# mhauskn/dqn-hfo

Hardware: AMD Instinct MI355X
Metric: DQN updates/sec, 1v0 HFO, 4x1024 MLP, minibatch 256 (higher is better)
Workload: dtype f32; 1 GPU; BASELINE configs[1]: 1v0 HFO, 1 MI355X, 4x1024 actor-critic, minibatch 256, 1M-transition device replay; replay_transitions=1000000, state_size=58, minibatch=256, minibatch_per_gpu=256, global_minibatch=256, parallelism=single, hip_graph=True, prewarm_updates=992, tuning_flags=0, sampling=on-device Philox, uniform with replacement

## Files before the change

### dqn-hfo_amd/capi.py

```python
import ctypes as C
import os

from ._build import LIB, build

MAX_HIDDEN = 8
DP_ID_BYTES = 128
DP_PER_LAYER, DP_HALF_GRADS, DP_SHARD_OPT = 1, 2, 4
DP_UNVERIFIED_OK = 256
TUNE_FP16_WGRAD_PER_LAYER = 1
TUNE_SEPARATE_HEAD_SEED = 2
TUNE_BWD_UNSHIFTED = 4
TUNE_SEPARATE_ACTOR_HEAD_BWD = 8
TUNE_SEPARATE_Q_TRAIN = 16
TUNE_SEPARATE_FIRST_LAYER = 32
TUNE_SEPARATE_CRITIC_FIRST_LAYERS = 64
TUNE_LATE_GATHER = 128
PLAN_FORMS = ("fp16", "data_parallel", "bwd_shifted_critic", "bwd_shifted_actor", "head_wgrad_rides_critic", "head_wgrad_rides_actor",
              "q_train_in_dgrad", "head_seed_fused", "dqda_head_bwd", "critic_l0_rides", "first_layers_merged", "early_gather_l0", "dp_tails_ride", "prioritized")
LOSS_SCALE_STATIC, LOSS_SCALE_DYNAMIC = 0, 1
FP32, FP16 = 0, 1
ACTOR, CRITIC, ACTOR_TARGET, CRITIC_TARGET = 0, 1, 2, 3
KIND_W, KIND_M, KIND_V, KIND_G = 0, 1, 2, 3
SOLVERS = ("Adam", "SGD", "Nesterov", "AdaGrad", "RMSProp", "AdaDelta")


class Config(C.Structure):
    _fields_ = [
        ("struct_size", C.c_int32), ("minibatch", C.c_int32), ("state_size", C.c_int32),
        ("num_hidden", C.c_int32), ("hidden", C.c_int32 * MAX_HIDDEN),
        ("replay_capacity", C.c_int32), ("soft_update_freq", C.c_int32),
        ("gamma", C.c_double), ("beta", C.c_double), ("tau", C.c_double),
        ("actor_lr", C.c_float), ("critic_lr", C.c_float), ("momentum", C.c_float),
        ("momentum2", C.c_float), ("delta", C.c_float), ("clip_gradients", C.c_float),
        ("device", C.c_int32), ("dp_world", C.c_int32), ("dp_rank", C.c_int32), ("use_graph", C.c_int32),
        ("seed", C.c_uint64), ("stream", C.c_void_p), ("grad_arena", C.c_void_p),
        ("grad_arena_bytes", C.c_size_t), ("precision", C.c_int32), ("loss_scale", C.c_float),
        ("solver_type", C.c_int32), ("rms_decay", C.c_float),
        ("tuning_flags", C.c_int32),
        ("loss_scale_mode", C.c_int32), ("loss_scale_growth_interval", C.c_int32),
        ("loss_scale_min_mult", C.c_float), ("loss_scale_max_mult", C.c_float),
    ]


class LossScaleState(C.Structure):
    _fields_ = [("struct_size", C.c_int32), ("mode", C.c_int32), ("mult_critic", C.c_float), ("mult_actor", C.c_float),
                ("good_critic", C.c_int32), ("good_actor", C.c_int32), ("backoffs_critic", C.c_int32), ("backoffs_actor", C.c_int32),
                ("growths_critic", C.c_int32), ("growths_actor", C.c_int32), ("skipped_steps", C.c_int32), ("reserved", C.c_int32)]


class UpdatePlan(C.Structure):
    _fields_ = [("struct_size", C.c_int32), ("forms", C.c_int32), ("launches_single", C.c_int32), ("launches_graph_first", C.c_int32),
                ("launches_in_graph", C.c_int32), ("updates_per_graph", C.c_int32), ("collectives", C.c_int32), ("solver_type", C.c_int32)]


class PerConfig(C.Structure):
    _fields_ = [("struct_size", C.c_int32), ("alpha", C.c_float), ("beta0", C.c_float), ("beta_anneal_iters", C.c_int32),
                ("eps", C.c_float), ("seed", C.c_uint64)]


class PerState(C.Structure):
    _fields_ = [("struct_size", C.c_int32), ("enabled", C.c_int32), ("levels", C.c_int32), ("size", C.c_int32),
                ("total", C.c_float), ("p_max", C.c_float), ("beta_now", C.c_float), ("reserved", C.c_float),
                ("next_counter", C.c_uint64), ("syncs", C.c_int64)]


class StateInfo(C.Structure):
    _fields_ = [("struct_size", C.c_int32), ("version", C.c_int32), ("flags", C.c_int32), ("precision", C.c_int32), ("minibatch", C.c_int32),
                ("state_size", C.c_int32), ("num_hidden", C.c_int32), ("hidden", C.c_int32 * MAX_HIDDEN), ("replay_capacity", C.c_int32),
                ("memory_size", C.c_int32), ("actor_iter", C.c_int32), ("critic_iter", C.c_int32), ("has_memory", C.c_int32),
                ("has_per", C.c_int32), ("has_loss_scale", C.c_int32), ("seed", C.c_uint64), ("update_counter", C.c_uint64),
                ("user_bytes", C.c_uint64), ("file_bytes", C.c_uint64), ("solver_type", C.c_int32), ("rms_decay", C.c_float)]


STATE_NO_MEMORY = 1

DIAG_BINS = 64
DIAG_MAX_BLOBS = 2 * (2 * MAX_HIDDEN + 4)
DIAG_MAX_PANELS = 5 * MAX_HIDDEN


class DiagMoments(C.Structure):
    _fields_ = [("count", C.c_int64), ("n_zero", C.c_int64), ("n_nonfinite", C.c_int64), ("sum_abs", C.c_double), ("sum_sq", C.c_double),
                ("max_abs", C.c_float), ("reserved", C.c_float)]


class DiagBlob(C.Structure):
    _fields_ = [("net", C.c_int32), ("layer", C.c_int32), ("is_bias", C.c_int32), ("reserved", C.c_int32),
                ("w", DiagMoments), ("g", DiagMoments), ("lag", DiagMoments), ("step", DiagMoments), ("g_hist", C.c_int32 * DIAG_BINS)]


class DiagPanel(C.Structure):
    _fields_ = [("pass_", C.c_int32), ("layer", C.c_int32), ("rows", C.c_int32), ("cols", C.c_int32), ("n_negative", C.c_int64),
                ("dead_units", C.c_int32), ("reserved", C.c_int32), ("a", DiagMoments), ("hist", C.c_int32 * DIAG_BINS)]


class DiagRow(C.Structure):
    _fields_ = [("min", C.c_float), ("max", C.c_float), ("sum", C.c_double), ("sum_sq", C.c_double), ("n_nonfinite", C.c_int64)]


class DiagAction(C.Structure):
    _fields_ = [("min", C.c_float), ("max", C.c_float), ("sum", C.c_double), ("n_out_of_bounds", C.c_int64)]


class DiagReport(C.Structure):
    _fields_ = [("struct_size", C.c_int32), ("n_blobs", C.c_int32), ("n_panels", C.c_int32), ("has_per", C.c_int32),
                ("blobs", DiagBlob * DIAG_MAX_BLOBS), ("panels", DiagPanel * DIAG_MAX_PANELS),
                ("q_target", DiagRow), ("y", DiagRow), ("q_train", DiagRow), ("q_policy", DiagRow), ("td", DiagRow),
                ("n_terminal", C.c_int64), ("actor_out", DiagAction * 10),
                ("dq_da_sum_abs", C.c_double), ("dq_da_max_abs", C.c_float), ("per_w_min", C.c_float), ("per_w_sum", C.c_double),
                ("per_prob_min", C.c_float), ("per_td_abs_max", C.c_float), ("actor_iter", C.c_int32), ("critic_iter", C.c_int32),
                ("critic_loss", C.c_float), ("avg_q", C.c_float), ("grad_norm", C.c_double * 2), ("clip_scale", C.c_double * 2),
                ("fp16", C.c_int32), ("loss_scale_mode", C.c_int32), ("loss_scale_critic", C.c_float), ("loss_scale_dqda", C.c_float),
                ("loss_scale_actor", C.c_float), ("mult_critic", C.c_float), ("mult_actor", C.c_float), ("reserved", C.c_int32)]

fp = C.POINTER(C.c_float)
ip = C.POINTER(C.c_int32)
up = C.POINTER(C.c_uint8)
H = C.c_void_p

SIGNATURES = {
    "dqnhip_default_config": (None, [C.POINTER(Config), C.c_int32]),
    "dqnhip_solver_name": (C.c_char_p, [C.c_int32]),
    "dqnhip_grad_arena_bytes": (C.c_size_t, [C.POINTER(Config)]),
    "dqnhip_last_error": (C.c_char_p, []),
    "dqnhip_create": (C.c_int, [C.POINTER(Config), C.POINTER(H)]),
    "dqnhip_destroy": (C.c_int, [H]),
    "dqnhip_update": (C.c_int, [H, ip, fp, fp]),
    "dqnhip_update_chained": (C.c_int, [H, ip, ip, fp, fp]),
    "dqnhip_update_async": (C.c_int, [H, ip]),
    "dqnhip_update_async_n": (C.c_int, [H, C.c_int32]),
    "dqnhip_update_pipelined": (C.c_int, [H, ip, fp, fp]),
    "dqnhip_update_indexed_n": (C.c_int, [H, ip, C.c_int32]),
    "dqnhip_collect_stats": (C.c_int, [H, fp, fp, C.c_int32, ip]),
    "dqnhip_benchmark_blocking": (C.c_int, [H, C.c_int32, C.c_int32, C.c_uint64, C.c_int32, fp]),
    "dqnhip_update_phase": (C.c_int, [H, C.c_int32, ip]),
    "dqnhip_update_abort": (C.c_int, [H]),
    "dqnhip_apply_update": (C.c_int, [H, C.c_int32]),
    "dqnhip_apply_update_sharded": (C.c_int, [H, C.c_int32, C.c_int32]),
    "dqnhip_get_update_plan": (C.c_int, [H, C.POINTER(UpdatePlan)]),
    "dqnhip_grad_buffer": (C.c_int, [H, C.c_int32, C.POINTER(C.c_void_p), C.POINTER(C.c_size_t)]),
    "dqnhip_read_stats": (C.c_int, [H, fp, fp]),
    "dqnhip_dp_unique_id": (C.c_int, [C.c_void_p, C.c_size_t]),
    "dqnhip_dp_init": (C.c_int, [H, C.c_void_p, C.c_size_t, C.c_int32]),
    "dqnhip_dp_init_file": (C.c_int, [H, C.c_char_p, C.c_int32, C.c_int32]),
    "dqnhip_dp_rendezvous_file": (C.c_int, [C.c_char_p, C.c_int32, C.c_int32, C.c_int32, C.c_void_p, C.c_size_t]),
    "dqnhip_dp_rendezvous_cleanup": (C.c_int, [C.c_char_p, C.c_int32]),
    "dqnhip_dp_graph_active": (C.c_int, [H, ip]),
    "dqnhip_dp_broadcast_params": (C.c_int, [H, C.c_int32]),
    "dqnhip_dp_update": (C.c_int, [H, ip]),
    "dqnhip_dp_update_n": (C.c_int, [H, C.c_int32]),
    "dqnhip_dp_gather_state": (C.c_int, [H]),
    "dqnhip_dp_destroy": (C.c_int, [H]),
    "dqnhip_dp_info": (C.c_int, [ip, C.c_char_p, C.c_size_t]),
    "dqnhip_skipped_steps": (C.c_int, [H, C.POINTER(C.c_int64)]),
    "dqnhip_get_loss_scale": (C.c_int, [H, C.POINTER(LossScaleState)]),
    "dqnhip_set_loss_scale": (C.c_int, [H, C.c_float, C.c_float]),
    "dqnhip_reduce_gradients_local": (C.c_int, [C.POINTER(H), C.c_int32, C.c_int32]),
    "dqnhip_sample_states": (C.c_int, [H, ip, C.c_int32, fp]),
    "dqnhip_get_actor_output": (C.c_int, [H, C.c_int32, C.c_int32, fp]),
    "dqnhip_files_matching_regexp": (C.c_int, [C.c_char_p, C.c_char_p, C.c_size_t, ip]),
    "dqnhip_remove_snapshots": (C.c_int, [C.c_char_p, C.c_int32]),
    "dqnhip_benchmark": (C.c_int, [H, C.c_int32, C.c_int32, fp]),
    "dqnhip_select_actions": (C.c_int, [H, fp, C.c_int32, fp]),
    "dqnhip_select_actions_device": (C.c_int, [H, C.c_void_p, C.c_int32, C.c_void_p]),
    "dqnhip_select_actions_net": (C.c_int, [H, C.c_int32, fp, C.c_int32, fp]),
    "dqnhip_critic_forward": (C.c_int, [H, C.c_int32, fp, fp, C.c_int32, fp]),
    "dqnhip_set_act_precision": (C.c_int, [H, C.c_int32]),
    "dqnhip_get_act_precision": (C.c_int, [H, ip]),
    "dqnhip_add_transitions": (C.c_int, [H, fp, fp, fp, fp, fp, up, C.c_int32]),
    "dqnhip_add_transition": (C.c_int, [H, fp, fp, C.c_float, C.c_float, fp, C.c_uint8]),
    "dqnhip_add_transitions_device": (C.c_int, [H, C.c_void_p, C.c_void_p, C.c_void_p, C.c_void_p,
                                                C.c_void_p, C.c_void_p, C.c_int32]),
    "dqnhip_label_transitions": (C.c_int, [C.c_double, fp, C.c_int32, fp]),
    "dqnhip_memory_size": (C.c_int, [H, ip]),
    "dqnhip_clear_memory": (C.c_int, [H]),
    "dqnhip_read_memory": (C.c_int, [H, C.c_int32, C.c_int32, fp, fp, fp, fp, fp, up]),
    "dqnhip_snapshot_replay_memory": (C.c_int, [H, C.c_char_p]),
    "dqnhip_load_replay_memory": (C.c_int, [H, C.c_char_p]),
    "dqnhip_get_config": (C.c_int, [H, C.POINTER(Config)]),
    "dqnhip_save_caffemodel": (C.c_int, [H, C.c_int32, C.c_char_p]),
    "dqnhip_load_caffemodel": (C.c_int, [H, C.c_int32, C.c_char_p]),
    "dqnhip_solver_snapshot": (C.c_int, [H, C.c_int32, C.c_char_p, ip]),
    "dqnhip_solver_restore": (C.c_int, [H, C.c_int32, C.c_char_p]),
    "dqnhip_snapshot": (C.c_int, [H, C.c_char_p, C.c_char_p, C.c_int32, C.c_int32]),
    "dqnhip_snapshot_async": (C.c_int, [H, C.c_char_p, C.c_char_p, C.c_int32, C.c_int32, C.c_int32]),
    "dqnhip_snapshot_wait": (C.c_int, [H, C.POINTER(C.c_int32), C.POINTER(C.c_int32)]),
    "dqnhip_snapshot_poll": (C.c_int, [H, C.POINTER(C.c_int32)]),
    "dqnhip_find_latest_snapshot": (C.c_int, [C.c_char_p, C.c_char_p, C.c_char_p, C.c_char_p, C.c_size_t]),
    "dqnhip_find_hiscore": (C.c_int, [C.c_char_p, ip]),
    "dqnhip_remove_files_matching_regexp": (C.c_int, [C.c_char_p]),
    "dqnhip_param_count": (C.c_int, [H, C.c_int32, C.POINTER(C.c_size_t)]),
    "dqnhip_get_params": (C.c_int, [H, C.c_int32, C.c_int32, fp, C.c_size_t]),
    "dqnhip_set_params": (C.c_int, [H, C.c_int32, C.c_int32, fp, C.c_size_t]),
    "dqnhip_clone_to_target": (C.c_int, [H, C.c_int32]),
    "dqnhip_share_parameters": (C.c_int, [H, H, C.c_int32, C.c_int32]),
    "dqnhip_share_replay_memory": (C.c_int, [H, H]),
    "dqnhip_get_iters": (C.c_int, [H, ip, ip]),
    "dqnhip_set_iters": (C.c_int, [H, C.c_int32, C.c_int32]),
    "dqnhip_debug_read": (C.c_int, [H, C.c_char_p, fp, C.c_size_t]),
    "dqnhip_get_stream": (C.c_int, [H, C.POINTER(C.c_void_p)]),
    "dqnhip_set_kernel_timing": (C.c_int, [H, C.c_int32]),
    "dqnhip_get_kernel_timing": (C.c_int, [H, C.c_char_p, fp, C.POINTER(C.c_int64), C.c_int32]),
    "dqnhip_diag_collect": (C.c_int, [H, C.POINTER(DiagReport)]),
    "dqnhip_per_default_config": (None, [C.POINTER(PerConfig)]),
    "dqnhip_per_enable": (C.c_int, [H, C.POINTER(PerConfig)]),
    "dqnhip_per_get_state": (C.c_int, [H, C.POINTER(PerState)]),
    "dqnhip_per_get_priorities": (C.c_int, [H, C.c_int32, C.c_int32, fp]),
    "dqnhip_per_set_priorities": (C.c_int, [H, C.c_int32, C.c_int32, fp]),
    "dqnhip_per_sample": (C.c_int, [H, C.c_uint64, C.c_int32, ip, fp]),
    "dqnhip_per_debug_read": (C.c_int, [H, C.c_char_p, fp, C.c_size_t]),
    "dqnhip_save_state": (C.c_int, [H, C.c_char_p, C.c_int32, C.c_void_p, C.c_size_t]),
    "dqnhip_load_state": (C.c_int, [H, C.c_char_p]),
    "dqnhip_state_info": (C.c_int, [C.c_char_p, C.POINTER(StateInfo)]),
    "dqnhip_state_read_user": (C.c_int, [C.c_char_p, C.c_void_p, C.c_size_t, C.POINTER(C.c_size_t)]),
    "dqnhip_save_state_async": (C.c_int, [H, C.c_char_p, C.c_int32, C.c_void_p, C.c_size_t]),
    "dqnhip_save_state_wait": (C.c_int, [H]),
    "dqnhip_save_state_poll": (C.c_int, [H, C.POINTER(C.c_int32)]),
    "dqnhip_state_crc32_device": (C.c_int, [H, C.c_void_p, C.c_size_t, C.c_int32, C.POINTER(C.c_uint32)]),
}

class EnvConfig(C.Structure):
    _fields_ = [("struct_size", C.c_int32), ("workers", C.c_int32), ("max_steps", C.c_int32), ("unum", C.c_int32),
                ("p_end", C.c_float), ("p_goal", C.c_float), ("seed", C.c_uint64)]


SIGNATURES.update({
    "dqnhip_env_create": (C.c_int, [H, C.POINTER(EnvConfig), C.POINTER(C.c_void_p)]),
    "dqnhip_env_destroy": (C.c_int, [C.c_void_p]),
    "dqnhip_env_step": (C.c_int, [C.c_void_p, C.c_float, C.c_int32]),
    "dqnhip_env_stats": (C.c_int, [C.c_void_p, C.POINTER(C.c_int64), C.POINTER(C.c_int64), C.POINTER(C.c_double),
                                   C.POINTER(C.c_int64)]),
    "dqnhip_env_debug_read": (C.c_int, [C.c_void_p, C.c_char_p, fp, C.c_size_t]),
})

ENV_NO_RECORD = 1


class EnvEpisode(C.Structure):
    _fields_ = [("total_reward", C.c_double), ("extrinsic_reward", C.c_double), ("steps", C.c_int32), ("status", C.c_int32),
                ("worker", C.c_int32), ("reserved", C.c_int32), ("step_index", C.c_int64)]


SIGNATURES.update({
    "dqnhip_env_create_external": (C.c_int, [H, C.POINTER(EnvConfig), C.c_int32, fp, C.POINTER(C.c_void_p)]),
    "dqnhip_env_act": (C.c_int, [C.c_void_p, C.c_float, ip, fp, fp]),
    "dqnhip_env_act_device": (C.c_int, [C.c_void_p, C.c_float, C.c_void_p, C.c_void_p, C.c_void_p]),
    "dqnhip_env_observe": (C.c_int, [C.c_void_p, fp, ip, ip]),
    "dqnhip_env_observe_device": (C.c_int, [C.c_void_p, C.c_void_p, C.c_void_p, C.c_void_p]),
    "dqnhip_env_read_episodes": (C.c_int, [C.c_void_p, C.POINTER(EnvEpisode), C.c_int32, ip, C.POINTER(C.c_int64)]),
})

_lib = None


def load(rebuild=False):
    global _lib
    if _lib is None or rebuild:
        build()
        if not os.path.exists(LIB):
            raise RuntimeError("libdqnhip.so is missing: the HIP extension is mandatory")
        lib = C.CDLL(LIB)
        for name, (res, args) in SIGNATURES.items():
            fn = getattr(lib, name)
            fn.restype = res
            fn.argtypes = args
        _lib = lib
    return _lib
```

### dqn-hfo_amd/csrc/gemm_bodies.hip.h

```cpp
#pragma once
#include <hip/hip_runtime.h>

#include <cstdint>

#include "learner_args.hip.h"

namespace dqnhip {


__host__ __device__ __forceinline__ void tile_of_counts(int tiles_p, int tiles_q, int b, int& tile_p, int& tile_q) {
  const bool xmap = (tiles_p & 7) == 0;
  const int j = xmap ? b >> 3 : b;
  const int d = j / tiles_q;
  tile_q = j - d * tiles_q;
  tile_p = xmap ? d * 8 + (b & 7) : d;
}
constexpr int kTileDecodeMaxQ = 1024, kTileDecodeMaxTiles = 1 << 18;
__host__ __device__ __forceinline__ uint32_t tile_magic(int tiles_q) { return (uint32_t)((0x80000000ull + (uint32_t)tiles_q - 1) / (uint32_t)tiles_q); }
__host__ __device__ __forceinline__ bool tile_magic_covers(int tiles_p, int tiles_q) {
  return tiles_p >= 1 && tiles_q >= 1 && tiles_q <= kTileDecodeMaxQ && (int64_t)tiles_p * tiles_q <= kTileDecodeMaxTiles;
}
__host__ __device__ __forceinline__ void tile_decode(int tiles_p, int tiles_q, uint32_t magic, int b, int& tile_p, int& tile_q) {
  const bool xmap = (tiles_p & 7) == 0;
  const int j = xmap ? b >> 3 : b;
  const int d = (int)(((uint64_t)(2u * (uint32_t)j + 1u) * magic) >> 32);
  tile_q = j - d * tiles_q;
  tile_p = xmap ? d * 8 + (b & 7) : d;
}
__device__ __forceinline__ void tile_of_problem(const GemmProblem& pr, int b, int& tile_p, int& tile_q) {
  tile_of_counts(pr.tiles_p, pr.tiles_q, b, tile_p, tile_q);
}
__device__ __forceinline__ void tile_of_block(const GemmBatch& batch, int& pi, int& tile_p, int& tile_q) {
  int b = blockIdx.x;
  pi = 0;
#pragma unroll
  for (int i = 1; i < kMaxGroup; ++i)
    if (i < batch.n && b >= batch.prob[i].tile_base) pi = i;
  const GemmProblem& pr = batch.prob[pi];
  tile_of_problem(pr, b - pr.tile_base, tile_p, tile_q);
}

__device__ __forceinline__ GemmProblem make_problem(const float* P, const float* Q, float* C, int ldp, int ldq, int ldc, int Pdim, int Qdim, int Kred,
                                                    int mode, const GemmCold& c, int tiles_p, int tiles_q, int tile_base) {
  GemmProblem pr;
  pr.P = P; pr.ldp = ldp; pr.Q = Q; pr.ldq = ldq; pr.C = C; pr.ldc = ldc; pr.Pdim = Pdim; pr.Qdim = Qdim; pr.Kred = Kred;
  pr.bias = c.bias; pr.mask = c.mask; pr.ldm = c.ldm; pr.db = c.db; pr.partial = c.partial; pr.relu = c.relu;
  pr.seed_w = c.seed_w; pr.C2 = c.C2; pr.dot_w = c.dot_w; pr.dot_out = c.dot_out;
  pr.xcopy_dst = c.xcopy_dst; pr.xcopy_col = c.xcopy_col; pr.xcopy_n = c.xcopy_n;
  pr.mode = mode; pr.tiles_p = tiles_p; pr.tiles_q = tiles_q; pr.tile_base = tile_base;
  return pr;
}
template <int N>
struct HotArgs { GemmHeader hd; GemmHot hot[N]; };
template <int N>
__device__ __forceinline__ int request_args(const GemmArgs<N>& a, HotArgs<N>& r, int b, int x0 = 0, int x1 = 0) {
  r.hd = a.head;
#pragma unroll
  for (int i = 0; i < N; ++i) r.hot[i] = a.hot[i];
  const GemmHot &h0 = r.hot[0], &h1 = r.hot[N > 1 ? 1 : 0], &h2 = r.hot[N > 2 ? 2 : 0], &h3 = r.hot[N > 3 ? 3 : 0];
  asm volatile("" : "+s"(b) : "s"(r.hd.tile_base[1]), "s"(r.hd.tiles_p[0]), "s"(r.hd.tiles_q[0]), "s"(x0), "s"(x1),
               "s"(h0.P), "s"(h0.ldp), "s"(h0.C), "s"(h1.P), "s"(h1.ldp), "s"(h1.C), "s"(h2.P), "s"(h2.ldp), "s"(h2.C), "s"(h3.P), "s"(h3.ldp), "s"(h3.C),
               "s"(h0.Pdim), "s"(h1.Pdim), "s"(h2.Pdim), "s"(h3.Pdim), "s"(h0.tq_magic), "s"(h1.tq_magic), "s"(h2.tq_magic), "s"(h3.tq_magic));
  return b;
}
template <int I, int N>
__device__ __forceinline__ GemmProblem problem_at(const GemmArgs<N>& a, const HotArgs<N>& r) {
  static_assert(I < N, "record not carried");
  const GemmHot& h = r.hot[I];
  return make_problem(h.P, h.Q, h.C, h.ldp, h.ldq, h.ldc, h.Pdim, h.Qdim, h.Kred, h.mode, a.cold[I], r.hd.tiles_p[I], r.hd.tiles_q[I], r.hd.tile_base[I]);
}
template <int I, int N>
__device__ __forceinline__ void tile_of_record(const HotArgs<N>& r, int b, int& tile_p, int& tile_q) {
  static_assert(I < N, "record not carried");
  tile_decode(r.hd.tiles_p[I], r.hd.tiles_q[I], r.hot[I].tq_magic, b, tile_p, tile_q);
}
template <int N>
__device__ __forceinline__ GemmProblem problem_of_tile(const GemmArgs<N>& a, const HotArgs<N>& r, const int b, int& tile_p, int& tile_q) {
  const GemmHeader& hd = r.hd;
  int pi = 0;
  int tiles_p = hd.tiles_p[0], tiles_q = hd.tiles_q[0], tile_base = hd.tile_base[0];
  GemmHot h = r.hot[0];
  if (N > 1 && b >= hd.tile_base[N > 1 ? 1 : 0]) {
    pi = 1;
    tiles_p = hd.tiles_p[N > 1 ? 1 : 0]; tiles_q = hd.tiles_q[N > 1 ? 1 : 0]; tile_base = hd.tile_base[N > 1 ? 1 : 0];
    h = r.hot[N > 1 ? 1 : 0];
    if (N > 2 && b >= hd.tile_base[N > 2 ? 2 : 0]) {
      constexpr int I2 = N > 2 ? 2 : 0, I3 = N > 3 ? 3 : I2;
      const bool last = N > 3 && b >= hd.tile_base[I3];
      const GemmHot &h2 = r.hot[I2], &h3 = r.hot[I3];
      pi = last ? I3 : I2;
      tiles_p = last ? hd.tiles_p[I3] : hd.tiles_p[I2]; tiles_q = last ? hd.tiles_q[I3] : hd.tiles_q[I2];
      tile_base = last ? hd.tile_base[I3] : hd.tile_base[I2];
      h.P = last ? h3.P : h2.P; h.Q = last ? h3.Q : h2.Q; h.C = last ? h3.C : h2.C;
      h.ldp = last ? h3.ldp : h2.ldp; h.ldq = last ? h3.ldq : h2.ldq; h.ldc = last ? h3.ldc : h2.ldc;
      h.Pdim = last ? h3.Pdim : h2.Pdim; h.Qdim = last ? h3.Qdim : h2.Qdim; h.Kred = last ? h3.Kred : h2.Kred;
      h.mode = last ? h3.mode : h2.mode; h.tq_magic = last ? h3.tq_magic : h2.tq_magic;
      asm volatile("" : "+s"(pi));
    }
    asm volatile("" : "+s"(pi));
  }
  tile_decode(tiles_p, tiles_q, h.tq_magic, b - tile_base, tile_p, tile_q);
  return make_problem(h.P, h.Q, h.C, h.ldp, h.ldq, h.ldc, h.Pdim, h.Qdim, h.Kred, h.mode, a.cold[N == 1 ? 0 : pi], tiles_p, tiles_q, tile_base);
}
template <int N>
__device__ __forceinline__ GemmProblem problem_of_block(const GemmArgs<N>& a, int& tile_p, int& tile_q) {
  HotArgs<N> r;
  const int b = request_args(a, r, (int)blockIdx.x);
  return problem_of_tile(a, r, b, tile_p, tile_q);
}

template <int NACC>
__device__ __forceinline__ void park_accumulators(float* smem, const f32x4 (&acc)[NACC], int wave, int lane) {
  f32x4* s = reinterpret_cast<f32x4*>(smem);
#pragma unroll
  for (int e = 0; e < NACC; ++e) s[(wave * NACC + e) * 64 + lane] = acc[e];
}
template <int NACC>
__device__ __forceinline__ f32x4 reduce_accumulator(const float* smem, int e, int lane) {
  const f32x4* s = reinterpret_cast<const f32x4*>(smem);
  const f32x4 a0 = s[(0 * NACC + e) * 64 + lane], a1 = s[(1 * NACC + e) * 64 + lane];
  const f32x4 a2 = s[(2 * NACC + e) * 64 + lane], a3 = s[(3 * NACC + e) * 64 + lane];
  f32x4 r;
  r.x = (a0.x + a1.x) + (a2.x + a3.x); r.y = (a0.y + a1.y) + (a2.y + a3.y);
  r.z = (a0.z + a1.z) + (a2.z + a3.z); r.w = (a0.w + a1.w) + (a2.w + a3.w);
  return r;
}

#define DQN_MFMA(a, b, c) __builtin_amdgcn_mfma_f32_16x16x4f32((a), (b), (c), 0, 0, 0)
#define DQN_PIN() __builtin_amdgcn_sched_barrier(0)

__device__ __forceinline__ void store_head_seed(const GemmProblem& pr, int q, int p, const f32x4& v, const f32x4& sw) {
  f32x4 dz;
  dz.x = (-sw.x) * lrelu_mask(v.x); dz.y = (-sw.y) * lrelu_mask(v.y);
  dz.z = (-sw.z) * lrelu_mask(v.z); dz.w = (-sw.w) * lrelu_mask(v.w);
  *reinterpret_cast<f32x4*>(pr.C2 + (size_t)q * pr.ldc + p) = dz;
}

__device__ __forceinline__ void store_head_dot(const GemmProblem& pr, int q, int p, int lg, const f32x4& v, const f32x4& dw) {
  float d = fmaf(v.x, dw.x, 0.0f); d = fmaf(v.y, dw.y, d); d = fmaf(v.z, dw.z, d); d = fmaf(v.w, dw.w, d);
  d += __shfl_xor(d, 16, 64);
  d += __shfl_xor(d, 32, 64);
  if (lg == 0) pr.dot_out[(size_t)q * (pr.Pdim >> 4) + (p >> 4)] = d;
}

template <int TP, int TQ>
__device__ __forceinline__ void fwd_direct_body(const GemmProblem& pr, int tile_p, int tile_q, float* smem) {
  constexpr int NACC = TP * TQ;
  const int lane = threadIdx.x & 63, wave = threadIdx.x >> 6;
  const int li = lane & 15, lg = lane >> 4;
  const int p0 = tile_p * 16 * TP, q0 = tile_q * 16 * TQ;
  const int Kw = pr.Kred >> 2;
  const int nkb = Kw >> 4;
  const int wave_u = __builtin_amdgcn_readfirstlane(wave);
  const char* pp[TP];
  const char* qp[TQ];
  const uint32_t lofp = ((uint32_t)li * (uint32_t)pr.ldp + (uint32_t)lg * 4u) * 4u, lofq = ((uint32_t)li * (uint32_t)pr.ldq + (uint32_t)lg * 4u) * 4u;
#pragma unroll
  for (int c = 0; c < TP; ++c) pp[c] = c == 0 ? reinterpret_cast<const char*>(pr.P + (size_t)p0 * pr.ldp + wave_u * Kw) : pp[c > 0 ? c - 1 : 0] + (size_t)64 * pr.ldp;
#pragma unroll
  for (int a = 0; a < TQ; ++a) qp[a] = a == 0 ? reinterpret_cast<const char*>(pr.Q + (size_t)q0 * pr.ldq + wave_u * Kw) : qp[a > 0 ? a - 1 : 0] + (size_t)64 * pr.ldq;

  f32x4 acc[NACC];
#pragma unroll
  for (int e = 0; e < NACC; ++e) acc[e] = f32x4{0.f, 0.f, 0.f, 0.f};
  f32x4 rp[4][TP], rq[4][TQ];

#define FWD_LOAD(slot, kb)                                                              \
  {                                                                                     \
    _Pragma("unroll") for (int c = 0; c < TP; ++c)                                      \
        rp[slot][c] = *reinterpret_cast<const f32x4*>(pp[c] + ((kb) << 6) + lofp);     \
    _Pragma("unroll") for (int a = 0; a < TQ; ++a)                                      \
        rq[slot][a] = *reinterpret_cast<const f32x4*>(qp[a] + ((kb) << 6) + lofq);     \
  }
#define FWD_COMPUTE(slot)                                                               \
  {                                                                                     \
    _Pragma("unroll") for (int s = 0; s < 4; ++s)                                       \
    _Pragma("unroll") for (int a = 0; a < TQ; ++a)                                      \
    _Pragma("unroll") for (int c = 0; c < TP; ++c)                                      \
        acc[a * TP + c] = DQN_MFMA(rp[slot][c][s], rq[slot][a][s], acc[a * TP + c]);    \
  }

  const int nkb4 = nkb & ~3;
  if (nkb4 > 0) {
    FWD_LOAD(0, 0) FWD_LOAD(1, 1) FWD_LOAD(2, 2) FWD_LOAD(3, 3)
    int kb = 0;
    for (; kb + 4 < nkb4; kb += 4) {
      FWD_COMPUTE(0) DQN_PIN(); FWD_LOAD(0, kb + 4) DQN_PIN();
      FWD_COMPUTE(1) DQN_PIN(); FWD_LOAD(1, kb + 5) DQN_PIN();
      FWD_COMPUTE(2) DQN_PIN(); FWD_LOAD(2, kb + 6) DQN_PIN();
      FWD_COMPUTE(3) DQN_PIN(); FWD_LOAD(3, kb + 7) DQN_PIN();
    }
    FWD_COMPUTE(0) FWD_COMPUTE(1) FWD_COMPUTE(2) FWD_COMPUTE(3)
  }
  {
    const int rem = nkb - nkb4;
    if (rem > 0) FWD_LOAD(0, nkb4)
    if (rem > 1) FWD_LOAD(1, nkb4 + 1)
    if (rem > 2) FWD_LOAD(2, nkb4 + 2)
    if (rem > 0) FWD_COMPUTE(0)
    if (rem > 1) FWD_COMPUTE(1)
    if (rem > 2) FWD_COMPUTE(2)
  }
#undef FWD_LOAD
#undef FWD_COMPUTE

  constexpr int NBV = (NACC + 3) / 4;
  f32x4 bvp[NBV], swp[NBV], dwp[NBV];
  if (pr.bias != nullptr) {
#pragma unroll
    for (int j = 0; j < NBV; ++j) {
      const int e = j * 4 + wave;
      if (e < NACC) bvp[j] = *reinterpret_cast<const f32x4*>(pr.bias + p0 + (e % TP) * 16 + (lg << 2));
    }
  }
  if (pr.seed_w != nullptr) {
#pragma unroll
    for (int j = 0; j < NBV; ++j) {
      const int e = j * 4 + wave;
      if (e < NACC) swp[j] = *reinterpret_cast<const f32x4*>(pr.seed_w + p0 + (e % TP) * 16 + (lg << 2));
    }
  }
  if (pr.dot_w != nullptr) {
#pragma unroll
    for (int j = 0; j < NBV; ++j) {
      const int e = j * 4 + wave;
      if (e < NACC) dwp[j] = *reinterpret_cast<const f32x4*>(pr.dot_w + p0 + (e % TP) * 16 + (lg << 2));
    }
  }
  if (pr.xcopy_dst != nullptr && (int)threadIdx.x < 16 * TP) {
    const float* src = pr.P + (size_t)(p0 + threadIdx.x) * pr.ldp + pr.xcopy_col;
    for (int j = tile_q; j < pr.xcopy_n; j += pr.tiles_q) pr.xcopy_dst[(size_t)j * pr.Pdim + p0 + threadIdx.x] = src[j];
  }
  park_accumulators<NACC>(smem, acc, wave, lane);
  __syncthreads();
#pragma unroll
  for (int e = 0; e < NACC; ++e) {
    if ((e & 3) == wave) {
      const int a = e / TP, c = e % TP;
      f32x4 v = reduce_accumulator<NACC>(smem, e, lane);
      const int q = q0 + a * 16 + li, p = p0 + c * 16 + (lg << 2);
      if (pr.bias != nullptr) {
        const f32x4 bv = bvp[e >> 2];
        v.x += bv.x; v.y += bv.y; v.z += bv.z; v.w += bv.w;
      }
      if (pr.relu) { v.x = lrelu_fwd(v.x); v.y = lrelu_fwd(v.y); v.z = lrelu_fwd(v.z); v.w = lrelu_fwd(v.w); }
      *reinterpret_cast<f32x4*>(pr.C + (size_t)q * pr.ldc + p) = v;
      if (pr.seed_w != nullptr) store_head_seed(pr, q, p, v, swp[e >> 2]);
      if (pr.dot_w != nullptr) store_head_dot(pr, q, p, lg, v, dwp[e >> 2]);
    }
  }
}

template <int TPB, int TQ>
__device__ __forceinline__ void dgrad_direct_body(const GemmProblem& pr, int tile_p, int tile_q, float* smem) {
  constexpr int NACC = TPB * 4 * TQ;
  const int lane = threadIdx.x & 63, wave = threadIdx.x >> 6;
  const int li = lane & 15, lg = lane >> 4;
  const int p0 = tile_p * 64 * TPB, q0 = tile_q * 16 * TQ;
  const int Kw = pr.Kred >> 2;
  const int nkb = Kw >> 4;
  const float* pp = pr.P + (size_t)(wave * Kw + lg * 4) * pr.ldp + p0 + li * 4;
  const float* qp[TQ];
#pragma unroll
  for (int a = 0; a < TQ; ++a) qp[a] = pr.Q + (size_t)(q0 + a * 16 + li) * pr.ldq + wave * Kw + lg * 4;
  const size_t ldp = pr.ldp;

  f32x4 acc[NACC];
#pragma unroll
  for (int e = 0; e < NACC; ++e) acc[e] = f32x4{0.f, 0.f, 0.f, 0.f};
  f32x4 rp[4][4][TPB], rq[4][TQ];

#define DG_LOAD(slot, kb)                                                               \
  {                                                                                     \
    _Pragma("unroll") for (int a = 0; a < TQ; ++a)                                      \
        rq[slot][a] = *reinterpret_cast<const f32x4*>(qp[a] + ((kb) << 4));            \
    _Pragma("unroll") for (int s = 0; s < 4; ++s)                                       \
    _Pragma("unroll") for (int b = 0; b < TPB; ++b)                                     \
        rp[slot][s][b] = *reinterpret_cast<const f32x4*>(pp + (size_t)(((kb) << 4) + s) * ldp + b * 64); \
  }
#define DG_COMPUTE(slot)                                                                \
  {                                                                                     \
    _Pragma("unroll") for (int s = 0; s < 4; ++s)                                       \
    _Pragma("unroll") for (int a = 0; a < TQ; ++a)                                      \
    _Pragma("unroll") for (int b = 0; b < TPB; ++b)                                     \
    _Pragma("unroll") for (int pc = 0; pc < 4; ++pc)                                    \
        acc[(a * TPB + b) * 4 + pc] =                                                   \
            DQN_MFMA(rp[slot][s][b][pc], rq[slot][a][s], acc[(a * TPB + b) * 4 + pc]);  \
  }

  const int nkb4 = nkb & ~3;
  if (nkb4 > 0) {
    DG_LOAD(0, 0) DG_LOAD(1, 1) DG_LOAD(2, 2) DG_LOAD(3, 3)
    int kb = 0;
    for (; kb + 4 < nkb4; kb += 4) {
      DG_COMPUTE(0) DQN_PIN(); DG_LOAD(0, kb + 4) DQN_PIN();
      DG_COMPUTE(1) DQN_PIN(); DG_LOAD(1, kb + 5) DQN_PIN();
      DG_COMPUTE(2) DQN_PIN(); DG_LOAD(2, kb + 6) DQN_PIN();
      DG_COMPUTE(3) DQN_PIN(); DG_LOAD(3, kb + 7) DQN_PIN();
    }
    DG_COMPUTE(0) DG_COMPUTE(1) DG_COMPUTE(2) DG_COMPUTE(3)
  }
  for (int kb = nkb4; kb < nkb; ++kb) { DG_LOAD(0, kb) DG_COMPUTE(0) }
#undef DG_LOAD
#undef DG_COMPUTE

  constexpr int NMK = (TQ * TPB + 3) / 4;
  f32x4 mk[NMK][4];
  if (pr.mask != nullptr) {
#pragma unroll
    for (int j = 0; j < NMK; ++j) {
      const int ab = j * 4 + wave;
      if (ab < TQ * TPB) {
#pragma unroll
        for (int r = 0; r < 4; ++r)
          mk[j][r] = *reinterpret_cast<const f32x4*>(pr.mask + (size_t)(q0 + (ab / TPB) * 16 + li) * pr.ldm + p0 + (ab % TPB) * 64 + (lg << 4) + (r << 2));
      }
    }
  }
  park_accumulators<NACC>(smem, acc, wave, lane);
  __syncthreads();
#pragma unroll
  for (int ab = 0; ab < TQ * TPB; ++ab) {
    if ((ab & 3) == wave) {
      const int a = ab / TPB, b = ab % TPB;
      f32x4 r0 = reduce_accumulator<NACC>(smem, ab * 4 + 0, lane);
      f32x4 r1 = reduce_accumulator<NACC>(smem, ab * 4 + 1, lane);
      f32x4 r2 = reduce_accumulator<NACC>(smem, ab * 4 + 2, lane);
      f32x4 r3 = reduce_accumulator<NACC>(smem, ab * 4 + 3, lane);
      const int q = q0 + a * 16 + li;
#pragma unroll
      for (int r = 0; r < 4; ++r) {
        const int p = p0 + b * 64 + (lg << 4) + (r << 2);
        f32x4 v = f32x4{r0[r], r1[r], r2[r], r3[r]};
        if (pr.mask != nullptr) {
          const f32x4 mv = mk[ab >> 2][r];
          v.x *= lrelu_mask(mv.x); v.y *= lrelu_mask(mv.y); v.z *= lrelu_mask(mv.z); v.w *= lrelu_mask(mv.w);
        }
        *reinterpret_cast<f32x4*>(pr.C + (size_t)q * pr.ldc + p) = v;
      }
    }
  }
}

template <int NS = 4>
__device__ __forceinline__ f32x4 dgrad_narrow_tile(const GemmProblem& pr, int tile_p, int tile_q, float* smem) {
  constexpr int NACC = 1;
  const int lane = threadIdx.x & 63, wave = threadIdx.x >> 6;
  const int li = lane & 15, lg = lane >> 4;
  const int p0 = tile_p * 16, q0 = tile_q * 16;
  const int Kw = pr.Kred >> 2;
  const int nkb = Kw >> 4;
  const float* pp = pr.P + (size_t)(wave * Kw + lg * 4) * pr.ldp + p0 + li;
  const float* qp = pr.Q + (size_t)(q0 + li) * pr.ldq + wave * Kw + lg * 4;
  const size_t ldp = pr.ldp;
  f32x4 acc[NACC];
  acc[0] = f32x4{0.f, 0.f, 0.f, 0.f};
  float rp[NS][4]; f32x4 rq[NS];
#define DN_LOAD(slot, kb)                                                               \
  {                                                                                     \
    rq[slot] = *reinterpret_cast<const f32x4*>(qp + ((kb) << 4));                      \
    _Pragma("unroll") for (int s = 0; s < 4; ++s) rp[slot][s] = pp[(size_t)(((kb) << 4) + s) * ldp]; \
  }
#define DN_COMPUTE(slot)                                                                \
  { _Pragma("unroll") for (int s = 0; s < 4; ++s) acc[0] = DQN_MFMA(rp[slot][s], rq[slot][s], acc[0]); }
  const int nkbN = nkb - nkb % NS;
  if (nkbN > 0) {
#pragma unroll
    for (int i = 0; i < NS; ++i) { DN_LOAD(i, i) DQN_PIN(); }
    int kb = 0;
    for (; kb + NS < nkbN; kb += NS) {
#pragma unroll
      for (int i = 0; i < NS; ++i) { DN_COMPUTE(i) DQN_PIN(); DN_LOAD(i, kb + NS + i) DQN_PIN(); }
    }
#pragma unroll
    for (int i = 0; i < NS; ++i) { DN_COMPUTE(i) }
  }
  for (int kb = nkbN; kb < nkb; ++kb) { DN_LOAD(0, kb) DN_COMPUTE(0) }
#undef DN_LOAD
#undef DN_COMPUTE
  f32x4 mv = f32x4{0.f, 0.f, 0.f, 0.f};
  if (wave == 0 && pr.mask != nullptr) mv = *reinterpret_cast<const f32x4*>(pr.mask + (size_t)(q0 + li) * pr.ldm + p0 + (lg << 2));
  park_accumulators<NACC>(smem, acc, wave, lane);
  __syncthreads();
  f32x4 v = f32x4{0.f, 0.f, 0.f, 0.f};
  if (wave == 0) {
    v = reduce_accumulator<NACC>(smem, 0, lane);
    if (pr.mask != nullptr) {
      v.x *= lrelu_mask(mv.x); v.y *= lrelu_mask(mv.y); v.z *= lrelu_mask(mv.z); v.w *= lrelu_mask(mv.w);
    }
  }
  return v;
}
template <int NS = 4>
__device__ __forceinline__ f32x4 dgrad_narrow_tile16(const NarrowTile16& pr, int tile_q, float* smem) {
  typedef __attribute__((ext_vector_type(4))) _Float16 h4;
  const int lane = threadIdx.x & 63, wave = threadIdx.x >> 6;
  const int li = lane & 15, lg = lane >> 4;
  const int q0 = tile_q * 16;
  const int Kw = pr.Kred >> 2;
  const int nkb = Kw >> 4;
  const _Float16* pp = pr.P + (size_t)(wave * Kw + lg * 4) * pr.ldp + li;
  const _Float16* qp = pr.Q + (size_t)(q0 + li) * pr.ldq + wave * Kw + lg * 4;
  const size_t ldp = pr.ldp;
  f32x4 acc[1];
  acc[0] = f32x4{0.f, 0.f, 0.f, 0.f};
  _Float16 rp[NS][4]; h4 rq[NS];
#define DN_LOAD(slot, kb)                                                               \
  {                                                                                     \
    rq[slot] = *reinterpret_cast<const h4*>(qp + ((kb) << 4));                         \
    _Pragma("unroll") for (int s = 0; s < 4; ++s) rp[slot][s] = pp[(size_t)(((kb) << 4) + s) * ldp]; \
  }
// ... 617 lines not shown
```

### dqn-hfo_amd/csrc/gemm_common.hip.h

```cpp
#pragma once
#include <hip/hip_runtime.h>
#include <hip/hip_ext.h>
#include <stdint.h>

namespace dqnhip {

typedef float f32x4 __attribute__((ext_vector_type(4)));

enum GemmMode { GEMM_FWD = 0, GEMM_DGRAD = 1, GEMM_WGRAD = 2 };

constexpr float kLeakySlope = 0.01f;

struct GemmProblem {
  const float* P; int ldp;
  const float* Q; int ldq;
  float* C; int ldc;
  int Pdim, Qdim, Kred;
  const float* bias;
  const float* mask; int ldm;
  float* db;
  float* partial;
  int relu;
  const float* seed_w; float* C2;
  const float* dot_w; float* dot_out;
  float* xcopy_dst; int xcopy_col, xcopy_n;
  int mode;
  int tiles_p, tiles_q, tile_base;
};

constexpr int kMaxLeadingDim = 1 << 26;
constexpr int kMaxGroup = 4;
struct GemmBatch {
  GemmProblem prob[kMaxGroup];
  int n;
  int total_tiles;
};

struct alignas(64) GemmHeader {
  int tile_base[kMaxGroup];
  int tiles_p[kMaxGroup], tiles_q[kMaxGroup];
  int n, total_tiles, pad[2];
};
struct alignas(64) GemmHot {
  const float* P; const float* Q;
  int ldp, ldq, Kred, ldc;
  float* C;
  int mode;
  int Pdim, Qdim;
  uint32_t tq_magic;
  int pad[2];
};
struct GemmCold {
  const float* bias; const float* mask; float* db; float* partial;
  const float* seed_w; float* C2; const float* dot_w; float* dot_out; float* xcopy_dst;
  int ldm, relu, xcopy_col, xcopy_n;
};
template <int N>
struct GemmArgs {
  GemmHeader head;
  GemmHot hot[N];
  GemmCold cold[N];
};
static_assert(sizeof(GemmHeader) == 64 && sizeof(GemmHot) == 64, "one 16-dword scalar load each");

struct LaunchOn {
  hipStream_t stream;
  hipEvent_t start = nullptr, stop = nullptr;
  LaunchOn(hipStream_t s) : stream(s) {}
  LaunchOn(hipStream_t s, hipEvent_t t0, hipEvent_t t1) : stream(s), start(t0), stop(t1) {}
};
template <typename K, typename... A>
inline hipError_t launch(const LaunchOn& on, K kernel, dim3 grid, dim3 block, size_t lds, const A&... args) {
  if (on.start) hipExtLaunchKernelGGL(kernel, grid, block, (uint32_t)lds, on.stream, on.start, on.stop, 0, args...);
  else hipLaunchKernelGGL(kernel, grid, block, lds, on.stream, args...);
  return hipGetLastError();
}

__device__ __forceinline__ float lrelu_fwd(float x) {
  return fmaxf(x, 0.0f) + kLeakySlope * fminf(x, 0.0f);
}
__device__ __forceinline__ float lrelu_mask(float y) {
  return (y > 0.0f ? 1.0f : 0.0f) + kLeakySlope * (y <= 0.0f ? 1.0f : 0.0f);
}

__device__ __forceinline__ float wave_sum64(float v) {
  v += __builtin_bit_cast(float, __builtin_amdgcn_update_dpp(0, __builtin_bit_cast(int, v), 0xB1, 0xF, 0xF, false));
  v += __builtin_bit_cast(float, __builtin_amdgcn_update_dpp(0, __builtin_bit_cast(int, v), 0x4E, 0xF, 0xF, false));
  v += __builtin_bit_cast(float, __builtin_amdgcn_update_dpp(0, __builtin_bit_cast(int, v), 0x141, 0xF, 0xF, false));
  v += __builtin_bit_cast(float, __builtin_amdgcn_update_dpp(0, __builtin_bit_cast(int, v), 0x140, 0xF, 0xF, false));
  v += __builtin_bit_cast(float, __builtin_amdgcn_update_dpp(0, __builtin_bit_cast(int, v), 0x142, 0xA, 0xF, false));
  v += __builtin_bit_cast(float, __builtin_amdgcn_update_dpp(0, __builtin_bit_cast(int, v), 0x143, 0xC, 0xF, false));
  return __builtin_bit_cast(float, __builtin_amdgcn_readlane(__builtin_bit_cast(int, v), 63));
}

constexpr int kFlagTarget = 1;
constexpr int kFlagGradNorm = 2;

__device__ __forceinline__ float ls_live(float base, const float* mult) { return mult != nullptr ? base * *mult : base; }

struct TailsArgs {
  const float* loss_partial; int n_loss; const double* q_partial; int n_q;
  float inv_batch; float* critic_tail; float* actor_tail; const int* flags;
  int on;
};
__device__ __forceinline__ void tails_block(const TailsArgs& a, float* sdot , double* sq ) {
  const int t = threadIdx.x;
  float dot = 0.0f; double qs = 0.0;
  if (a.critic_tail != nullptr) for (int i = t; i < a.n_loss; i += 256) dot += a.loss_partial[i];
  if (a.actor_tail != nullptr) for (int i = t; i < a.n_q; i += 256) qs += a.q_partial[i];
#pragma unroll
  for (int off = 32; off > 0; off >>= 1) { dot += __shfl_xor(dot, off, 64); qs += __shfl_xor(qs, off, 64); }
  if ((t & 63) == 0) { sdot[t >> 6] = dot; sq[t >> 6] = qs; }
  __syncthreads();
  if (t != 0) return;
  if (a.critic_tail != nullptr) {
    dot = (sdot[0] + sdot[1]) + (sdot[2] + sdot[3]);
    a.critic_tail[0] = dot * a.inv_batch / 2.0f;
    a.critic_tail[1] = 0.f; a.critic_tail[2] = (*a.flags & kFlagTarget) ? 1.0f : 0.f; a.critic_tail[3] = 0.f;
  }
  if (a.actor_tail != nullptr) {
    qs = (sq[0] + sq[1]) + (sq[2] + sq[3]);
    a.actor_tail[0] = 0.f; a.actor_tail[1] = (float)qs; a.actor_tail[2] = 0.f; a.actor_tail[3] = 0.f;
  }
}

}
```

### dqn-hfo_amd/csrc/gemm_direct.hip.h

```cpp
#pragma once
#include <hip/hip_runtime.h>

#include <algorithm>
#include <cstdint>
#include <cstdlib>

#include "gemm_bodies.hip.h"
#include "gemm_plan.hip.h"

namespace dqnhip {

template <int TP, int TQ>
__global__ __launch_bounds__(256) void gemm_fwd_direct(const GemmArgs<kMaxGroup> args) {
  extern __shared__ __attribute__((aligned(16))) float smem[];
  int tile_p, tile_q;
  const GemmProblem pr = problem_of_block(args, tile_p, tile_q);
  fwd_direct_body<TP, TQ>(pr, tile_p, tile_q, smem);
}
template <int TP, int TQ, bool PIN, int NSLOT = 2>
__global__ __launch_bounds__(256) void gemm_fwd_lds(const GemmArgs<kMaxGroup> args) {
  extern __shared__ __attribute__((aligned(16))) float smem[];
  int tile_p, tile_q;
  const GemmProblem pr = problem_of_block(args, tile_p, tile_q);
  fwd_lds_body<TP, TQ, PIN, NSLOT>(pr, tile_p, tile_q, smem);
}
template <int TPB, int TQ>
__global__ __launch_bounds__(256) void gemm_dgrad_direct(const GemmArgs<kMaxGroup> args) {
  extern __shared__ __attribute__((aligned(16))) float smem[];
  int tile_p, tile_q;
  const GemmProblem pr = problem_of_block(args, tile_p, tile_q);
  dgrad_direct_body<TPB, TQ>(pr, tile_p, tile_q, smem);
}
template <int TPB, int TQ, bool SCH = true>
__device__ __forceinline__ void dgrad_lds_body(const GemmProblem& pr, int tile_p, int tile_q, float* smem) {
  DgradNoHook none;
  dgrad_lds_body<TPB, TQ, SCH, DgradNoHook>(pr, tile_p, tile_q, smem, nullptr, none);
}
template <int TPB, int TQ>
__global__ __launch_bounds__(256) void gemm_dgrad_lds(const GemmArgs<kMaxGroup> args) {
  extern __shared__ __attribute__((aligned(16))) float smem[];
  int tile_p, tile_q;
  const GemmProblem pr = problem_of_block(args, tile_p, tile_q);
  dgrad_lds_body<TPB, TQ>(pr, tile_p, tile_q, smem);
}
template <int TPB, int TQB>
__global__ __launch_bounds__(256) void gemm_wgrad_direct(const GemmArgs<kMaxGroup> args) {
  extern __shared__ __attribute__((aligned(16))) float smem[];
  int tile_p, tile_q;
  const GemmProblem pr = problem_of_block(args, tile_p, tile_q);
  wgrad_direct_body<TPB, TQB>(pr, tile_p, tile_q, smem);
}
template <int UNUSED = 0>
__global__ __launch_bounds__(256) void gemm_dgrad_narrow(const GemmArgs<kMaxGroup> args) {
  extern __shared__ __attribute__((aligned(16))) float smem[];
  int tile_p, tile_q;
  const GemmProblem pr = problem_of_block(args, tile_p, tile_q);
  dgrad_narrow_body(pr, tile_p, tile_q, smem);
}
template <int UNUSED = 0>
__global__ __launch_bounds__(256) void gemm_dgrad_narrow_qrider(const GemmArgs<kMaxGroup> args, const QHeadRider rider) {
  extern __shared__ __attribute__((aligned(16))) float smem[];
  HotArgs<kMaxGroup> r;
  const int b = request_args(args, r, (int)blockIdx.x, args.head.total_tiles);
  if (b >= r.hd.total_tiles) { q_head_rider(rider, b - r.hd.total_tiles); return; }
  int tile_p, tile_q;
  const GemmProblem pr = problem_of_tile(args, r, b, tile_p, tile_q);
  dgrad_narrow_body(pr, tile_p, tile_q, smem);
}
template <int TPB>
__global__ __launch_bounds__(256) void gemm_wgrad_narrow(const GemmArgs<kMaxGroup> args) {
  extern __shared__ __attribute__((aligned(16))) float smem[];
  int tile_p, tile_q;
  const GemmProblem pr = problem_of_block(args, tile_p, tile_q);
  wgrad_narrow_body<TPB>(pr, tile_p, tile_q, smem);
}
template <int TQD = 1, bool DLDS = false>
__global__ __launch_bounds__(256) void gemm_bwd_pair_direct(const GemmArgs<kMaxGroup> args) {
  extern __shared__ __attribute__((aligned(16))) float smem[];
  int tile_p, tile_q;
  const GemmProblem pr = problem_of_block(args, tile_p, tile_q);
  if (pr.mode == GEMM_WGRAD) wgrad_direct_body<1, 1>(pr, tile_p, tile_q, smem);
  else if constexpr (DLDS) dgrad_lds_body<1, TQD, false>(pr, tile_p, tile_q, smem);
  else dgrad_direct_body<1, TQD>(pr, tile_p, tile_q, smem);
}

template <bool DLDS>
__device__ __forceinline__ void bwd_seq_block(const GemmArgs<2>& args, const int block, float* smem) {
  int tile_p, tile_q;
  HotArgs<2> r;
  const int b = request_args(args, r, block);
  const GemmProblem pw = problem_at<1>(args, r);
  if (b < pw.tiles_p * pw.tiles_q) {
    tile_of_record<1>(r, b, tile_p, tile_q);
    wgrad_direct_body<1, 1>(pw, tile_p, tile_q, smem);
  }
  __syncthreads();
  const GemmProblem pd = problem_at<0>(args, r);
  if (b < pd.tiles_p * pd.tiles_q) {
    tile_of_record<0>(r, b, tile_p, tile_q);
    if constexpr (DLDS) dgrad_lds_body<1, 1, true>(pd, tile_p, tile_q, smem);
    else dgrad_direct_body<1, 1>(pd, tile_p, tile_q, smem);
  }
}
template <bool DLDS>
__global__ __launch_bounds__(256) void gemm_bwd_seq(const GemmArgs<2> args) {
  extern __shared__ __attribute__((aligned(16))) float smem[];
  bwd_seq_block<DLDS>(args, (int)blockIdx.x, smem);
}

template <int NH>
__global__ __launch_bounds__(256) void gemm_wgrad_narrow_rider(const GemmArgs<kMaxGroup> args, const HeadWgradRider rider) {
  extern __shared__ __attribute__((aligned(16))) float smem[];
  HotArgs<kMaxGroup> r;
  const int b = request_args(args, r, (int)blockIdx.x, rider.blocks);
  if (b < rider.blocks) { head_wgrad_rider<NH>(rider, b, smem); return; }
  int tile_p, tile_q;
  const GemmProblem pr = problem_of_tile(args, r, b - rider.blocks, tile_p, tile_q);
  wgrad_narrow_body<1>(pr, tile_p, tile_q, smem);
}

template <int NH>
__global__ __launch_bounds__(256) void gemm_wgrad_tail(const GemmArgs<2> args, const HeadWgradRider rider, const TailsArgs tails) {
  extern __shared__ __attribute__((aligned(16))) float smem[];
  HotArgs<2> r;
  int blk = request_args(args, r, (int)blockIdx.x, tails.on, rider.blocks);
  int tile_p, tile_q;
  if (tails.on && blk == tails.on - 1) { tails_block(tails, smem, reinterpret_cast<double*>(smem + 8)); return; }
  if (blk < rider.blocks) { head_wgrad_rider<NH>(rider, blk, smem); return; }
  blk -= rider.blocks;
  const int n0 = r.hd.tiles_p[1] * r.hd.tiles_q[1];
  if (blk < n0) { const GemmProblem p0 = problem_at<1>(args, r); tile_of_record<1>(r, blk, tile_p, tile_q); wgrad_narrow_body<1>(p0, tile_p, tile_q, smem); return; }
  blk -= n0;
  const GemmProblem p1 = problem_at<0>(args, r);
  tile_of_record<0>(r, blk, tile_p, tile_q); wgrad_direct_body<1, 1>(p1, tile_p, tile_q, smem);
}


constexpr int kBwdTileLds = 4 * 16 * 64 * 16 + 4 * 16 * 16;
constexpr int kWgradTailLdsMax = 80 * 1024;

inline int tile_batch(GemmBatch& batch, int BP, int BQ) {
  int base = 0;
  for (int i = 0; i < batch.n; ++i) {
    GemmProblem& p = batch.prob[i];
    p.tiles_p = p.Pdim / BP;
    p.tiles_q = p.Qdim / BQ;
    p.tile_base = base;
    base += p.tiles_p * p.tiles_q;
  }
  return batch.total_tiles = base;
}
template <typename K>
inline hipError_t direct_launch(K kernel, GemmBatch& batch, int BP, int BQ, int lds_bytes, const LaunchOn& on) {
  return launch(on, kernel, dim3(tile_batch(batch, BP, BQ)), dim3(256), lds_bytes, batch);
}
template <int N>
inline bool pack_args(const GemmBatch& b, GemmArgs<N>& a, bool grouped = true) {
  a = GemmArgs<N>{};
  if (b.n < 1 || b.n > N) return false;
  a.head.n = b.n; a.head.total_tiles = b.total_tiles;
  int base = 0;
  for (int i = 0; i < kMaxGroup; ++i) {
    a.head.tile_base[i] = INT32_MAX; a.head.tiles_p[i] = 1; a.head.tiles_q[i] = 1;
    if (i >= b.n) continue;
    const GemmProblem& p = b.prob[i];
    if (p.tiles_p < 1 || p.tiles_q < 1 || p.tile_base != (grouped ? base : 0)) return false;
    if (p.ldp > kMaxLeadingDim || p.ldq > kMaxLeadingDim) return false;
    if (!tile_magic_covers(p.tiles_p, p.tiles_q)) return false;
    const int count = p.tiles_p * p.tiles_q;
    base += count;
    a.head.tile_base[i] = p.tile_base; a.head.tiles_p[i] = p.tiles_p; a.head.tiles_q[i] = p.tiles_q;
    GemmHot& h = a.hot[i];
    h.P = p.P; h.Q = p.Q; h.C = p.C; h.ldp = p.ldp; h.ldq = p.ldq; h.ldc = p.ldc; h.Pdim = p.Pdim; h.Qdim = p.Qdim; h.Kred = p.Kred; h.mode = p.mode;
    h.tq_magic = tile_magic(p.tiles_q);
    GemmCold& c = a.cold[i];
    c.bias = p.bias; c.mask = p.mask; c.db = p.db; c.partial = p.partial; c.seed_w = p.seed_w; c.C2 = p.C2; c.dot_w = p.dot_w; c.dot_out = p.dot_out;
    c.xcopy_dst = p.xcopy_dst; c.ldm = p.ldm; c.relu = p.relu; c.xcopy_col = p.xcopy_col; c.xcopy_n = p.xcopy_n;
  }
  return true;
}
template <typename K, typename... R>
inline hipError_t packed_launch(K kernel, const GemmBatch& batch, int extra, int lds_bytes, const LaunchOn& on, const R&... riders) {
  GemmArgs<kMaxGroup> args;
  if (!pack_args(batch, args)) return hipErrorInvalidValue;
  return launch(on, kernel, dim3(batch.total_tiles + extra), dim3(256), lds_bytes, args, riders...);
}
template <typename K>
inline hipError_t packed_launch(K kernel, GemmBatch& batch, int BP, int BQ, int lds_bytes, const LaunchOn& on) {
  tile_batch(batch, BP, BQ);
  return packed_launch(kernel, batch, 0, lds_bytes, on);
}

template <int TP, int TQ>
constexpr int fwd_direct_lds_bytes() { return 4 * TP * TQ * 64 * 16; }
template <int TP, int TQ>
inline hipError_t fwd_direct_launch(GemmBatch& b, const LaunchOn& on) {
  return packed_launch(gemm_fwd_direct<TP, TQ>, b, 16 * TP, 16 * TQ, fwd_direct_lds_bytes<TP, TQ>(), on);
}
template <int TP, int TQ, bool PIN, int NSLOT = 2>
constexpr int fwd_lds_bytes() {
  return 4 * 4 * ((NSLOT * (TP + TQ) * 512 > TP * TQ * 256) ? NSLOT * (TP + TQ) * 512 : TP * TQ * 256);
}
template <int TP, int TQ, bool PIN, int NSLOT = 2>
inline hipError_t fwd_lds_launch(GemmBatch& b, const LaunchOn& on) {
  return packed_launch(gemm_fwd_lds<TP, TQ, PIN, NSLOT>, b, 16 * TP, 16 * TQ, (fwd_lds_bytes<TP, TQ, PIN, NSLOT>()), on);
}
template <int TPB, int TQ>
constexpr int dgrad_direct_lds_bytes() { return 4 * TPB * 4 * TQ * 64 * 16; }
template <int TPB, int TQ>
inline hipError_t dgrad_direct_launch(GemmBatch& b, const LaunchOn& on) {
  return packed_launch(gemm_dgrad_direct<TPB, TQ>, b, 64 * TPB, 16 * TQ, dgrad_direct_lds_bytes<TPB, TQ>(), on);
}
template <int TPB, int TQ>
constexpr int dgrad_lds_bytes() { return 4 * ((2 * TQ * 512 > TPB * 4 * TQ * 256) ? 2 * TQ * 512 : TPB * 4 * TQ * 256) * 4; }
template <int TPB, int TQ>
inline hipError_t dgrad_lds_launch(GemmBatch& b, const LaunchOn& on) {
  return packed_launch(gemm_dgrad_lds<TPB, TQ>, b, 64 * TPB, 16 * TQ, dgrad_lds_bytes<TPB, TQ>(), on);
}
template <int TPB, int TQB>
inline hipError_t wgrad_direct_launch(GemmBatch& b, const LaunchOn& on) {
  return packed_launch(gemm_wgrad_direct<TPB, TQB>, b, 64 * TPB, 64 * TQB,
                       4 * TPB * 4 * TQB * 4 * 64 * 16 + 4 * TQB * 16 * 16, on);
}
template <int TQD, bool DLDS = false>
inline hipError_t bwd_pair_direct_launch(GemmBatch& batch, const LaunchOn& on) {
  int base = 0;
  for (int i = 0; i < batch.n; ++i) {
    GemmProblem& p = batch.prob[i];
    p.tiles_p = p.Pdim / 64;
    p.tiles_q = p.Qdim / (p.mode == GEMM_WGRAD ? 64 : 16 * TQD);
    p.tile_base = base;
    base += p.tiles_p * p.tiles_q;
  }
  batch.total_tiles = base;
  return packed_launch(gemm_bwd_pair_direct<TQD, DLDS>, batch, 0, kBwdTileLds, on);
}
constexpr int kNarrowDgradLds = 4 * 64 * 16;
inline hipError_t dgrad_narrow_launch(GemmBatch& b, const LaunchOn& on) {
  return packed_launch(gemm_dgrad_narrow<0>, b, 16, 16, kNarrowDgradLds, on);
}
inline hipError_t dgrad_narrow_qrider_launch(GemmBatch& batch, const QHeadRider& rider, const LaunchOn& on) {
  tile_batch(batch, 16, 16);
  return packed_launch(gemm_dgrad_narrow_qrider<0>, batch, rider.blocks, kNarrowDgradLds, on, rider);
}
template <int TPB>
constexpr int wgrad_narrow_lds_bytes() { return 4 * TPB * 4 * 64 * 16 + 4 * 16 * 4; }
template <int TPB>
inline hipError_t wgrad_narrow_launch(GemmBatch& b, const LaunchOn& on) {
  return packed_launch(gemm_wgrad_narrow<TPB>, b, 64 * TPB, 16, wgrad_narrow_lds_bytes<TPB>(), on);
}
template <int NH>
inline size_t head_rider_lds_bytes(const HeadWgradRider& rider) { return (size_t)(rider.rows * NH + 16 * NH * 16) * sizeof(float); }
template <int NH>
inline hipError_t wgrad_narrow_rider_launch(GemmBatch& batch, const HeadWgradRider& rider, const LaunchOn& on) {
  const size_t lds = std::max(head_rider_lds_bytes<NH>(rider), (size_t)wgrad_narrow_lds_bytes<1>());
  if (lds > 64 * 1024) return hipErrorInvalidValue;
  tile_batch(batch, 64, 16);
  return packed_launch(gemm_wgrad_narrow_rider<NH>, batch, rider.blocks, (int)lds, on, rider);
}
template <int NH>
inline hipError_t wgrad_tail_launch(GemmBatch& batch, const HeadWgradRider& rider, const LaunchOn& on, const TailsArgs* tails_in = nullptr) {
  TailsArgs tails{}; if (tails_in != nullptr) { tails = *tails_in; tails.on = 1; }
  GemmProblem& w1 = batch.prob[0]; GemmProblem& w0 = batch.prob[1];
  w1.tiles_p = w1.Pdim / 64; w1.tiles_q = w1.Qdim / 64; w1.tile_base = 0;
  w0.tiles_p = w0.Pdim / 64; w0.tiles_q = w0.Qdim / 16; w0.tile_base = w1.tiles_p * w1.tiles_q;
  const int grid = w0.tile_base + w0.tiles_p * w0.tiles_q + rider.blocks + (tails.on ? 1 : 0);
  batch.total_tiles = grid;
  if (tails.on) tails.on = grid;
  const size_t lds = std::max(rider.blocks ? head_rider_lds_bytes<NH>(rider) : (size_t)0, (size_t)kBwdTileLds);
  if (lds > (size_t)kWgradTailLdsMax) return hipErrorInvalidValue;
  GemmArgs<2> args;
  if (batch.n != 2 || !pack_args(batch, args)) return hipErrorInvalidValue;
  return launch(on, gemm_wgrad_tail<NH>, dim3(grid), dim3(256), lds, args, rider, tails);
}
template <bool DLDS>
inline hipError_t bwd_seq_launch(GemmBatch& batch, const LaunchOn& on) {
  GemmProblem& d = batch.prob[0]; GemmProblem& w = batch.prob[1];
  d.tiles_p = d.Pdim / 64; d.tiles_q = d.Qdim / 16; d.tile_base = 0;
  w.tiles_p = w.Pdim / 64; w.tiles_q = w.Qdim / 64; w.tile_base = 0;
  const int nd = d.tiles_p * d.tiles_q, nw = w.tiles_p * w.tiles_q;
  const int grid = nd > nw ? nd : nw;
  batch.total_tiles = grid;
  GemmArgs<2> args;
  if (batch.n != 2 || !pack_args(batch, args, false)) return hipErrorInvalidValue;
  return launch(on, gemm_bwd_seq<DLDS>, dim3(grid), dim3(256), kBwdTileLds, args);
}
template <int UNUSED = 0>
inline hipError_t gemm_form_launch(int form, GemmBatch& b, const LaunchOn& on, const HeadWgradRider* rider = nullptr, const TailsArgs* tails = nullptr) {
  if (!gemm_form_accepts(form, b)) return hipErrorInvalidValue;
  const bool tail = form == GEMM_FORM_WGRAD_TAIL_1 || form == GEMM_FORM_WGRAD_TAIL_NO;
  if (!tail && (rider != nullptr || tails != nullptr)) return hipErrorInvalidValue;
  const HeadWgradRider no_rider{};
  switch (form) {
    case GEMM_FORM_FWD_DIRECT_2x2: return fwd_direct_launch<2, 2>(b, on);
    case GEMM_FORM_FWD_DIRECT_4x2: return fwd_direct_launch<4, 2>(b, on);
    case GEMM_FORM_FWD_LDS_1x1: return fwd_lds_launch<1, 1, true>(b, on);
    case GEMM_FORM_FWD_LDS_2x2: return fwd_lds_launch<2, 2, true>(b, on);
    case GEMM_FORM_FWD_LDS_4x2: return fwd_lds_launch<4, 2, true>(b, on);
    case GEMM_FORM_FWD_LDS_4x2_ONE_IMAGE: return fwd_lds_launch<4, 2, true, 1>(b, on);
    case GEMM_FORM_DGRAD_DIRECT: return dgrad_direct_launch<1, 1>(b, on);
    case GEMM_FORM_DGRAD_LDS: return dgrad_lds_launch<1, 1>(b, on);
    case GEMM_FORM_DGRAD_NARROW: return dgrad_narrow_launch(b, on);
    case GEMM_FORM_WGRAD_NARROW: return wgrad_narrow_launch<1>(b, on);
    case GEMM_FORM_BWD_SEQ: return bwd_seq_launch<false>(b, on);
    case GEMM_FORM_BWD_SEQ_LDS: return bwd_seq_launch<true>(b, on);
    case GEMM_FORM_BWD_PAIR: return bwd_pair_direct_launch<1, false>(b, on);
    case GEMM_FORM_BWD_PAIR_LDS: return bwd_pair_direct_launch<1, true>(b, on);
    case GEMM_FORM_WGRAD_TAIL_1: return wgrad_tail_launch<1>(b, rider ? *rider : no_rider, on, tails);
    case GEMM_FORM_WGRAD_TAIL_NO: return wgrad_tail_launch<kNO>(b, rider ? *rider : no_rider, on, tails);
  }
  return hipErrorInvalidValue;
}
template <typename K>
inline hipError_t direct_prepare(K kernel, int lds_bytes) {
  return hipFuncSetAttribute(reinterpret_cast<const void*>(kernel), hipFuncAttributeMaxDynamicSharedMemorySize, lds_bytes);
}
template <int UNUSED = 0>
inline hipError_t direct_prepare_all() {
  hipError_t e = direct_prepare(gemm_bwd_seq<true>, kBwdTileLds);
  if (e == hipSuccess) e = direct_prepare(gemm_bwd_seq<false>, kBwdTileLds);
  if (e == hipSuccess) e = direct_prepare(gemm_wgrad_tail<1>, kWgradTailLdsMax);
  if (e == hipSuccess) e = direct_prepare(gemm_wgrad_tail<10>, kWgradTailLdsMax);
  if (e == hipSuccess) e = direct_prepare(gemm_bwd_pair_direct<1, true>, kBwdTileLds);
  if (e == hipSuccess) e = direct_prepare(gemm_bwd_pair_direct<1, false>, kBwdTileLds);
  if (e == hipSuccess) e = direct_prepare(gemm_fwd_lds<4, 2, true>, fwd_lds_bytes<4, 2, true>());
  return e;
}

}
```

### dqn-hfo_amd/csrc/head_fwd_kernels.hip.h

```cpp
#pragma once
#include "learner_internal.hip.h"
#include "update_bodies.hip.h"

namespace dqnhip {

template <int NH, int MODE, bool L1 = false>
__global__ __launch_bounds__(256) void k_head_fwd(HeadArgs2 a2) {
  const HeadArgs& a = a2.p[blockIdx.y];
  const int wave = threadIdx.x >> 6, lane = threadIdx.x & 63;
  __shared__ float s_acc[4][NH];
  const bool hoist = a.H <= 1024;
  const float bias_j = threadIdx.x < NH ? a.b[threadIdx.x] : 0.0f;
  f32x4 wreg[NH];
  if (hoist) {
#pragma unroll
    for (int j = 0; j < NH; ++j)
      wreg[j] = (threadIdx.x * 4 < a.H) ? *reinterpret_cast<const f32x4*>(a.W + (size_t)j * a.H + threadIdx.x * 4) : f32x4{0.f, 0.f, 0.f, 0.f};
  }
  constexpr bool kL1 = (L1 && MODE == HEAD_ACTOR && NH == kNO);
  __shared__ float s_mu[kAP];
  float l1w[kL1 ? 4 : 1][kL1 ? kNO : 1];
  f32x4 l1b = f32x4{0.f, 0.f, 0.f, 0.f};
  const bool l1_on = kL1 && a.l1_y != nullptr && (int)threadIdx.x * 4 < a.l1_n;
  if constexpr (kL1) {
    if (l1_on) {
#pragma unroll
      for (int j = 0; j < kNO; ++j) {
        const f32x4 w4 = *reinterpret_cast<const f32x4*>(a.l1_wt + (size_t)j * a.l1_n + threadIdx.x * 4);
        l1w[0][j] = w4.x; l1w[1][j] = w4.y; l1w[2][j] = w4.z; l1w[3][j] = w4.w;
      }
      l1b = *reinterpret_cast<const f32x4*>(a.l1_b + threadIdx.x * 4);
    }
  }
  for (int row = blockIdx.x; row < a.rows; row += gridDim.x) {
    float acc[NH];
#pragma unroll
    for (int j = 0; j < NH; ++j) acc[j] = 0.0f;
    const size_t x0 = (size_t)row * a.ldx;
    f32x4 zs = f32x4{0.f, 0.f, 0.f, 0.f};
    if constexpr (kL1) { if (l1_on) zs = *reinterpret_cast<const f32x4*>(a.l1_zs + (size_t)row * a.l1_ld + threadIdx.x * 4); }
    auto dots = [&](auto tag) {
      for (int k = threadIdx.x * 4; k < a.H; k += 1024) {
        const f32x4 xv = head_ld4t<decltype(tag)::value>(a.X, a.X16, x0 + k);
#pragma unroll
        for (int j = 0; j < NH; ++j) {
          const f32x4 wv = hoist ? wreg[j] : *reinterpret_cast<const f32x4*>(a.W + (size_t)j * a.H + k);
          acc[j] = fmaf(xv.x, wv.x, acc[j]); acc[j] = fmaf(xv.y, wv.y, acc[j]);
          acc[j] = fmaf(xv.z, wv.z, acc[j]); acc[j] = fmaf(xv.w, wv.w, acc[j]);
        }
      }
    };
    HEAD_DISPATCH(a.X16 != nullptr, dots);
#pragma unroll
    for (int j = 0; j < NH; ++j) {
      acc[j] = wave_sum64(acc[j]);
      if (lane == 0) s_acc[wave][j] = acc[j];
    }
    __syncthreads();
    if (threadIdx.x < kAP) {
      const int j = threadIdx.x;
      float v = 0.0f;
      if (j < NH) v = ((s_acc[0][j] + s_acc[1][j]) + (s_acc[2][j] + s_acc[3][j])) + bias_j;
      if constexpr (MODE == HEAD_ACTOR) {
        a.out16[(size_t)row * kAP + j] = v;
        if (a.xc != nullptr && j < NH) a.xc[(size_t)row * a.ldxc + a.xc_col + j] = v;
        if (a.xc16 != nullptr && j < NH) a.xc16[(size_t)row * a.ldxc16 + a.xc_col + j] = (_Float16)v;
        if constexpr (kL1) s_mu[j] = v;
      } else {
        if (j == 0) {
          a.q[row] = v;
          if constexpr (MODE == HEAD_Q_POLICY) a.qsum_partial[row] = (double)v;
        }
      }
    }
    __syncthreads();
    if constexpr (kL1) {
      if (a.l1_y != nullptr) {
        if (l1_on) {
          float o[4] = {zs.x, zs.y, zs.z, zs.w};
#pragma unroll
          for (int e = 0; e < 4; ++e) {
#pragma unroll
            for (int j = 0; j < kNO; ++j) o[e] = fmaf(l1w[e][j], s_mu[j], o[e]);
          }
          f32x4 y;
          y.x = lrelu_fwd(o[0] + l1b.x); y.y = lrelu_fwd(o[1] + l1b.y); y.z = lrelu_fwd(o[2] + l1b.z); y.w = lrelu_fwd(o[3] + l1b.w);
          *reinterpret_cast<f32x4*>(a.l1_y + (size_t)row * a.l1_ld + threadIdx.x * 4) = y;
        }
        __syncthreads();
      }
    }
  }
}

template <int NH, int MODE>
__global__ __launch_bounds__(256) void k_head_fwd_rows(HeadArgs2 a2) {
  const HeadArgs& a = a2.p[blockIdx.y];
  const int wave = threadIdx.x >> 6, lane = threadIdx.x & 63;
  const bool in16 = a.X16 != nullptr;
  auto kof = [&](int t) { return in16 ? lane * 8 + 512 * (t >> 1) + 4 * (t & 1) : lane * 4 + 256 * t; };
  f32x4 wreg[NH][4];
#pragma unroll
  for (int j = 0; j < NH; ++j)
#pragma unroll
    for (int t = 0; t < 4; ++t) {
      const int k = kof(t);
      wreg[j][t] = k < a.H ? *reinterpret_cast<const f32x4*>(a.W + (size_t)j * a.H + k) : f32x4{0.f, 0.f, 0.f, 0.f};
    }
  auto load_row = [&](int row, f32x4 (&v)[4]) {
    const size_t x0 = (size_t)row * a.ldx;
    if (in16) {
      typedef __attribute__((ext_vector_type(8))) _Float16 h8;
      h8 u[2];
#pragma unroll
      for (int q = 0; q < 2; ++q) {
        const int k = lane * 8 + 512 * q;
        if (k < a.H) u[q] = *reinterpret_cast<const h8*>(a.X16 + x0 + k);
        else { for (int e = 0; e < 8; ++e) u[q][e] = (_Float16)0.f; }
      }
#pragma unroll
      for (int q = 0; q < 2; ++q) {
        v[2 * q] = f32x4{(float)u[q][0], (float)u[q][1], (float)u[q][2], (float)u[q][3]};
        v[2 * q + 1] = f32x4{(float)u[q][4], (float)u[q][5], (float)u[q][6], (float)u[q][7]};
      }
    } else {
#pragma unroll
      for (int t = 0; t < 4; ++t) {
        const int k = lane * 4 + 256 * t;
        v[t] = k < a.H ? *reinterpret_cast<const f32x4*>(a.X + x0 + k) : f32x4{0.f, 0.f, 0.f, 0.f};
      }
    }
  };
  const int row_step = gridDim.x * 4;
  const float bias_l = lane < NH ? a.b[lane] : 0.0f;
  f32x4 xn[4];
  if ((int)(blockIdx.x * 4 + wave) < a.rows) load_row(blockIdx.x * 4 + wave, xn);
  for (int row = blockIdx.x * 4 + wave; row < a.rows; row += row_step) {
    f32x4 xv[4];
#pragma unroll
    for (int t = 0; t < 4; ++t) xv[t] = xn[t];
    if (row + row_step < a.rows) load_row(row + row_step, xn);
    float acc[NH];
#pragma unroll
    for (int j = 0; j < NH; ++j) {
      float s = 0.0f;
#pragma unroll
      for (int t = 0; t < 4; ++t) {
        s = fmaf(xv[t].x, wreg[j][t].x, s); s = fmaf(xv[t].y, wreg[j][t].y, s);
        s = fmaf(xv[t].z, wreg[j][t].z, s); s = fmaf(xv[t].w, wreg[j][t].w, s);
      }
      acc[j] = wave_sum64(s);
    }
    if (lane < kAP) {
      float v = 0.0f;
#pragma unroll
      for (int j = 0; j < NH; ++j) if (lane == j) v = acc[j] + bias_l;
      if constexpr (MODE == HEAD_ACTOR) {
        a.out16[(size_t)row * kAP + lane] = v;
        if (a.xc != nullptr && lane < NH) a.xc[(size_t)row * a.ldxc + a.xc_col + lane] = v;
        if (a.xc16 != nullptr && lane < NH) a.xc16[(size_t)row * a.ldxc16 + a.xc_col + lane] = (_Float16)v;
      } else {
        if (lane == 0) {
          a.q[row] = v;
          if constexpr (MODE == HEAD_Q_POLICY) a.qsum_partial[row] = (double)v;
        }
      }
    }
  }
}

}

namespace dqnhip_host {

template <int NH, int MODE>
int head_forward(H* h, hipStream_t st, const HeadArgs& a, const HeadArgs* b = nullptr) {
  HeadArgs2 a2{}; a2.p[0] = a; if (b) a2.p[1] = *b;
  if constexpr (NH > 1) {
    if (a.rows >= 1024 && a.H <= 1024 && a.H % 4 == 0) {
      HIPCHK(launch(st, k_head_fwd_rows<NH, MODE>, dim3(256, b ? 2 : 1), dim3(256), 0, a2));
      return 0;
    }
  }
  if (a.l1_y != nullptr || (b && b->l1_y != nullptr))
    HIPCHK(launch(st, k_head_fwd<NH, MODE, true>, dim3(std::min(a.rows, 1024), b ? 2 : 1), dim3(256), 0, a2));
  else
    HIPCHK(launch(st, k_head_fwd<NH, MODE, false>, dim3(std::min(a.rows, 1024), b ? 2 : 1), dim3(256), 0, a2));
  return 0;
}

}
```

### dqn-hfo_amd/csrc/head_kernels.hip.h

```cpp
#pragma once
#include "gemm_direct.hip.h"
#include "update_bodies.hip.h"

namespace dqnhip {

static __global__ __launch_bounds__(256) void k_head_q_train(HeadTrainArgs a) {
  const int wave = threadIdx.x >> 6, lane = threadIdx.x & 63;
  const int row = blockIdx.x * 4 + wave;
  __shared__ float s_part[4];
  float at = 0.0f, ao = 0.0f;
  float bt0 = 0.0f, b0 = 0.0f, r = 0.0f, mcv = 0.0f, tm = 0.0f;
  if (row < a.rows && lane == 0) { bt0 = a.bt[0]; b0 = a.b[0]; r = a.reward[row]; mcv = a.mc[row]; tm = a.term[row]; }
  if (row < a.rows) {
    const size_t x0 = (size_t)row * a.H;
    auto dots = [&](auto tag) {
      for (int k = lane * 4; k < a.H; k += 256) {
        const f32x4 v0 = head_ld4t<decltype(tag)::value>(a.Xt, a.Xt16, x0 + k), w0 = *reinterpret_cast<const f32x4*>(a.Wt + k);
        const f32x4 v1 = head_ld4t<decltype(tag)::value>(a.X, a.X16, x0 + k), w1 = *reinterpret_cast<const f32x4*>(a.W + k);
        at = fmaf(v0.x, w0.x, at); at = fmaf(v0.y, w0.y, at); at = fmaf(v0.z, w0.z, at); at = fmaf(v0.w, w0.w, at);
        ao = fmaf(v1.x, w1.x, ao); ao = fmaf(v1.y, w1.y, ao); ao = fmaf(v1.z, w1.z, ao); ao = fmaf(v1.w, w1.w, ao);
      }
    };
    HEAD_DISPATCH(a.X16 != nullptr, dots);
  }
  at = wave_sum64(at); ao = wave_sum64(ao);
  float d2 = 0.0f, dq_row = 0.0f;
  if (row < a.rows && lane == 0) {
    const float qt = at + bt0, q = ao + b0;
    a.q_target[row] = qt; a.q[row] = q;
    const float off_policy = tm != 0.0f ? r : (float)((double)r + a.gamma * (double)qt);
    const float target = (float)(a.beta * (double)mcv + (1 - a.beta) * (double)off_policy);
    a.y[row] = target;
    if (!isfinite(target)) atomicOr(&a.st->flags, kFlagTarget);
    const float d = q - target;
    dq_row = a.inv_batch * d;
    a.dq[row] = dq_row;
    d2 = d * d;
  }
  if ((a.dZ != nullptr || a.dZ16 != nullptr) && row < a.rows) {
    const float dqv = __shfl(dq_row, 0, 64);
    const size_t x0 = (size_t)row * a.H;
    const float sc16 = a.dZ16 != nullptr ? ls_live(a.scale16, a.ls_mult) : 0.0f;
    auto seed = [&](auto tag) {
      for (int k = lane * 4; k < a.H; k += 256) {
        const f32x4 xv = head_ld4t<decltype(tag)::value>(a.X, a.X16, x0 + k), wv = *reinterpret_cast<const f32x4*>(a.W + k);
        f32x4 dz;
        dz.x = (dqv * wv.x) * lrelu_mask(xv.x); dz.y = (dqv * wv.y) * lrelu_mask(xv.y);
        dz.z = (dqv * wv.z) * lrelu_mask(xv.z); dz.w = (dqv * wv.w) * lrelu_mask(xv.w);
        if constexpr (decltype(tag)::value)
          *reinterpret_cast<head_h4*>(a.dZ16 + x0 + k) = head_h4{(_Float16)(dz.x * sc16), (_Float16)(dz.y * sc16), (_Float16)(dz.z * sc16), (_Float16)(dz.w * sc16)};
        else
          *reinterpret_cast<f32x4*>(a.dZ + x0 + k) = dz;
      }
    };
    HEAD_DISPATCH(a.X16 != nullptr, seed);
  }
  if (lane == 0) s_part[wave] = d2;
  __syncthreads();
  if (threadIdx.x == 0) a.loss_partial[blockIdx.x] = ((s_part[0] + s_part[1]) + s_part[2]) + s_part[3];
}

__device__ __forceinline__ float per_beta_now(float beta0, int anneal, int critic_iter) {
  if (anneal <= 0) return beta0;
  return fminf(1.0f, beta0 + (1.0f - beta0) * ((float)critic_iter / (float)anneal));
}
static __global__ __launch_bounds__(256) void k_head_q_train_w(HeadTrainWArgs aw) {
  const HeadTrainArgs& a = aw.t;
  const int wave = threadIdx.x >> 6, lane = threadIdx.x & 63;
  const int row = blockIdx.x * 4 + wave;
  __shared__ float s_part[4];
  float at = 0.0f, ao = 0.0f;
  float bt0 = 0.0f, b0 = 0.0f, r = 0.0f, mcv = 0.0f, tm = 0.0f, pr = 1.0f;
  if (row < a.rows && lane == 0) { bt0 = a.bt[0]; b0 = a.b[0]; r = a.reward[row]; mcv = a.mc[row]; tm = a.term[row]; pr = aw.prob[row]; }
  float pmin = INFINITY;
  for (int j = lane; j < a.rows; j += 64) pmin = fminf(pmin, aw.prob[j]);
  if (row < a.rows) {
    const size_t x0 = (size_t)row * a.H;
    auto dots = [&](auto tag) {
      for (int k = lane * 4; k < a.H; k += 256) {
        const f32x4 v0 = head_ld4t<decltype(tag)::value>(a.Xt, a.Xt16, x0 + k), w0 = *reinterpret_cast<const f32x4*>(a.Wt + k);
        const f32x4 v1 = head_ld4t<decltype(tag)::value>(a.X, a.X16, x0 + k), w1 = *reinterpret_cast<const f32x4*>(a.W + k);
        at = fmaf(v0.x, w0.x, at); at = fmaf(v0.y, w0.y, at); at = fmaf(v0.z, w0.z, at); at = fmaf(v0.w, w0.w, at);
        ao = fmaf(v1.x, w1.x, ao); ao = fmaf(v1.y, w1.y, ao); ao = fmaf(v1.z, w1.z, ao); ao = fmaf(v1.w, w1.w, ao);
      }
    };
    HEAD_DISPATCH(a.X16 != nullptr, dots);
  }
  at = wave_sum64(at); ao = wave_sum64(ao);
#pragma unroll
  for (int off = 32; off > 0; off >>= 1) pmin = fminf(pmin, __shfl_xor(pmin, off, 64));
  float d2 = 0.0f, dq_row = 0.0f;
  if (row < a.rows && lane == 0) {
    const float qt = at + bt0, q = ao + b0;
    a.q_target[row] = qt; a.q[row] = q;
    const float off_policy = tm != 0.0f ? r : (float)((double)r + a.gamma * (double)qt);
    const float target = (float)(a.beta * (double)mcv + (1 - a.beta) * (double)off_policy);
    a.y[row] = target;
    if (!isfinite(target)) atomicOr(&a.st->flags, kFlagTarget);
    const float beta = per_beta_now(aw.beta0, aw.beta_anneal_iters, a.st->critic_iter);
    const float w = beta == 0.0f ? 1.0f : powf(__fdiv_rn(pmin, pr), beta);
    const float d = q - target;
    dq_row = (a.inv_batch * d) * w;
    a.dq[row] = dq_row;
    d2 = (d * d) * w;
    aw.w[row] = w; aw.td_abs[row] = fabsf(d);
  }
  if ((a.dZ != nullptr || a.dZ16 != nullptr) && row < a.rows) {
    const float dqv = __shfl(dq_row, 0, 64);
    const size_t x0 = (size_t)row * a.H;
    const float sc16 = a.dZ16 != nullptr ? ls_live(a.scale16, a.ls_mult) : 0.0f;
    auto seed = [&](auto tag) {
      for (int k = lane * 4; k < a.H; k += 256) {
        const f32x4 xv = head_ld4t<decltype(tag)::value>(a.X, a.X16, x0 + k), wv = *reinterpret_cast<const f32x4*>(a.W + k);
        f32x4 dz;
        dz.x = (dqv * wv.x) * lrelu_mask(xv.x); dz.y = (dqv * wv.y) * lrelu_mask(xv.y);
        dz.z = (dqv * wv.z) * lrelu_mask(xv.z); dz.w = (dqv * wv.w) * lrelu_mask(xv.w);
        if constexpr (decltype(tag)::value)
          *reinterpret_cast<head_h4*>(a.dZ16 + x0 + k) = head_h4{(_Float16)(dz.x * sc16), (_Float16)(dz.y * sc16), (_Float16)(dz.z * sc16), (_Float16)(dz.w * sc16)};
        else
          *reinterpret_cast<f32x4*>(a.dZ + x0 + k) = dz;
      }
    };
    HEAD_DISPATCH(a.X16 != nullptr, seed);
  }
  if (lane == 0) s_part[wave] = d2;
  __syncthreads();
  if (threadIdx.x == 0) a.loss_partial[blockIdx.x] = ((s_part[0] + s_part[1]) + s_part[2]) + s_part[3];
}

struct QTrainHook {
  const HeadTrainArgs& a; float* s_scale; float* s_dq; int q0; bool owner;
  float v0[4], v1[4];
  float rw[4], mcv[4], tm[4], bt0, b0;
  f32x4 xv, wv;
  int c_first;
  __device__ __forceinline__ QTrainHook(const HeadTrainArgs& a_, float* sc, float* sd, int q0_, int tile_p) : a(a_), s_scale(sc), s_dq(sd), q0(q0_), owner(tile_p == 0), c_first(tile_p * 64) {}
  __device__ __forceinline__ void after_prologue() {
    const int lane = threadIdx.x & 63, wave = threadIdx.x >> 6;
    const int np = a.H >> 4;
    const int pc = lane < np ? lane : 0;
#pragma unroll
    for (int j = 0; j < 4; ++j) {
      const size_t x0 = (size_t)(q0 + wave * 4 + j) * np + pc;
      v0[j] = a.pdt[x0]; v1[j] = a.pd[x0];
      const int row = q0 + wave * 4 + j;
      rw[j] = a.reward[row]; mcv[j] = a.mc[row]; tm[j] = a.term[row];
    }
    bt0 = a.bt[0]; b0 = a.b[0];
    if (c_first < a.H) {
      const int rr = threadIdx.x >> 4, c = c_first + ((threadIdx.x & 15) << 2);
      xv = *reinterpret_cast<const f32x4*>(a.X + (size_t)(q0 + rr) * a.H + c); wv = *reinterpret_cast<const f32x4*>(a.W + c);
    }
  }
  __device__ __forceinline__ void before_park() {
    const int lane = threadIdx.x & 63, wave = threadIdx.x >> 6;
    const bool in = lane < (a.H >> 4);
    float d2[4];
#pragma unroll
    for (int j = 0; j < 4; ++j) {
      const int rr = wave * 4 + j, row = q0 + rr;
      const float at = wave_sum64(in ? v0[j] : 0.0f), ao = wave_sum64(in ? v1[j] : 0.0f);
      const float r = rw[j];
      const float qt = at + bt0, q = ao + b0;
      const float off_policy = tm[j] != 0.0f ? r : (float)((double)r + a.gamma * (double)qt);
      const float target = (float)(a.beta * (double)mcv[j] + (1 - a.beta) * (double)off_policy);
      const float d = q - target;
      const float dq_row = a.inv_batch * d;
      d2[j] = d * d;
      if (lane == 0) {
        s_scale[rr] = -dq_row; s_dq[rr] = dq_row;
        if (owner) {
          a.q_target[row] = qt; a.q[row] = q; a.y[row] = target; a.dq[row] = dq_row;
          if (!isfinite(target)) atomicOr(&a.st->flags, kFlagTarget);
        }
      }
    }
    if (owner && lane == 0) a.loss_partial[(q0 >> 2) + wave] = ((d2[0] + d2[1]) + d2[2]) + d2[3];
  }
};
template <int UNUSED = 0>
__global__ __launch_bounds__(256) __attribute__((amdgpu_waves_per_eu(1, 1))) void k_dgrad_qtrain(const GemmArgs<1> args, const HeadTrainArgs a) {
  extern __shared__ __attribute__((aligned(16))) float smem[];
  __shared__ float s_scale[16], s_dq[16];
  int tile_p, tile_q;
  HotArgs<1> r;
  const int b = request_args(args, r, (int)blockIdx.x);
  const GemmProblem pr = problem_at<0>(args, r);
  tile_of_record<0>(r, b, tile_p, tile_q);
  const int q0 = tile_q * 16;
  QTrainHook hook(a, s_scale, s_dq, q0, tile_p);
  dgrad_lds_body<1, 1, true, QTrainHook>(pr, tile_p, tile_q, smem, s_scale, hook);
  for (int c0 = tile_p * 64; c0 < a.H; c0 += pr.tiles_p * 64) {
    const int rr = threadIdx.x >> 4, c = c0 + ((threadIdx.x & 15) << 2);
    const size_t x0 = (size_t)(q0 + rr) * a.H + c;
    f32x4 xv = hook.xv, wv = hook.wv;
    if (c0 != tile_p * 64) { xv = *reinterpret_cast<const f32x4*>(a.X + x0); wv = *reinterpret_cast<const f32x4*>(a.W + c); }
    const float dqv = s_dq[rr];
    f32x4 dz;
    dz.x = (dqv * wv.x) * lrelu_mask(xv.x); dz.y = (dqv * wv.y) * lrelu_mask(xv.y);
    dz.z = (dqv * wv.z) * lrelu_mask(xv.z); dz.w = (dqv * wv.w) * lrelu_mask(xv.w);
    *reinterpret_cast<f32x4*>(a.dZ + x0) = dz;
  }
}
inline hipError_t dgrad_qtrain_launch(GemmBatch& batch, const HeadTrainArgs& a, const LaunchOn& on) {
  batch.n = 1;
  tile_batch(batch, 64, 16);
  GemmArgs<1> args;
  if (!pack_args(batch, args)) return hipErrorInvalidValue;
  return launch(on, k_dgrad_qtrain<0>, dim3(batch.total_tiles), dim3(256), dgrad_lds_bytes<1, 1>(), args, a);
}

__device__ __forceinline__ void slab_st(float* p, float v) { __hip_atomic_store(p, v, __ATOMIC_RELAXED, __HIP_MEMORY_SCOPE_AGENT); }
__device__ __forceinline__ float slab_ld(const float* p) { return __hip_atomic_load(p, __ATOMIC_RELAXED, __HIP_MEMORY_SCOPE_AGENT); }
template <int NH>
__global__ __launch_bounds__(1024) void k_head_bwd(HeadBwdArgs a) {
  extern __shared__ __attribute__((aligned(16))) float sm[];
  const int RC = a.rc_blocks > 0 ? a.rc_blocks : gridDim.y, rc = blockIdx.y, nkb = gridDim.x;
  if (a.q_out != nullptr && rc >= RC) {
    const int wave = threadIdx.x >> 6, lane = threadIdx.x & 63;
    const int row = (((int)blockIdx.y - RC) * (int)gridDim.x + (int)blockIdx.x) * 16 + wave;
    if (row >= a.rows) return;
    const float* rW = a.qr_W ? a.qr_W : a.W; const float* rX = a.qr_W ? a.qr_X4 : a.X4;
    const _Float16* rX16 = a.qr_W ? a.qr_X416 : a.X416; const int rH = a.qr_W ? a.qr_H : a.H;
    const size_t x0 = (size_t)row * rH;
    float acc = 0.0f;
    auto dots = [&](auto tag) {
      for (int k = lane * 4; k < rH; k += 256) {
        const f32x4 xv = head_ld4t<decltype(tag)::value>(rX, rX16, x0 + k), wv = *reinterpret_cast<const f32x4*>(rW + k);
        acc = fmaf(xv.x, wv.x, acc); acc = fmaf(xv.y, wv.y, acc); acc = fmaf(xv.z, wv.z, acc); acc = fmaf(xv.w, wv.w, acc);
      }
    };
    HEAD_DISPATCH(rX16 != nullptr, dots);
    acc = wave_sum64(acc);
    if (lane == 0) { const float v = acc + a.q_bias[0]; a.q_out[row] = v; a.qsum_partial[row] = (double)v; }
    return;
  }
  const int rows_c = (a.rows + RC - 1) / RC;
  const int r0 = rc * rows_c, r1 = min(a.rows, r0 + rows_c);
  float* s_dy = sm;
  float* s_acc = sm + rows_c * NH;
  __shared__ int s_last;
  const int tid = threadIdx.x;
  const bool want_w = a.dW != nullptr;
  const int kc = tid & 63, rg = tid >> 6;
  const int k = blockIdx.x * 64 + kc;
  const int per = (r1 - r0 + 15) / 16;
  const int m0 = r0 + rg * per, m1 = min(r1, m0 + per);
  constexpr int RB = 4;
  float w[NH];
#pragma unroll
  for (int j = 0; j < NH; ++j) w[j] = a.W[(size_t)j * a.H + k];
  float xpre[RB];
  auto ldx = [&](int m) -> float { return a.X416 != nullptr ? (float)a.X416[(size_t)m * a.H + k] : a.X4[(size_t)m * a.H + k]; };
#pragma unroll
  for (int u = 0; u < RB; ++u) xpre[u] = (m0 + u < m1) ? ldx(m0 + u) : 0.0f;
  for (int i = tid; i < (r1 - r0) * NH; i += 1024) {
    const int m = r0 + i / NH, j = i % NH;
    float d;
    if constexpr (NH == kNO) {
      d = a.dXc[(size_t)m * a.ldx + a.S + j];
      const float out = a.aout16[(size_t)m * kAP + j];
      float mn, mx;
      inverting_bounds(j, mn, mx);
      if (d < 0) d *= (mx - out) / (mx - mn);
      else if (d > 0) d *= (out - mn) / (mx - mn);
      if (blockIdx.x == 0) a.dA16[(size_t)m * kAP + j] = d;
    } else {
      d = a.dyh ? a.dyh[(size_t)m * a.lddy + j] : -1.0f;
    }
    s_dy[i] = d;
  }
  __syncthreads();
  float acc[NH];
#pragma unroll
  for (int j = 0; j < NH; ++j) acc[j] = 0.0f;
  const float sc16 = a.dZ16 != nullptr ? ls_live(a.scale16, a.ls_mult) : 0.0f;
  auto rows_loop = [&](auto tag) {
  for (int mb = m0; mb < m1; mb += RB) {
    float xb[RB];
#pragma unroll
    for (int u = 0; u < RB; ++u)
      xb[u] = (mb == m0) ? xpre[u] : ((mb + u < m1) ? head_ld1t<decltype(tag)::value>(a.X4, a.X416, (size_t)(mb + u) * a.H + k) : 0.0f);
#pragma unroll
    for (int u = 0; u < RB; ++u) {
      const int m = mb + u;
      if (m >= m1) break;
      const float xv = xb[u];
      float s0 = 0.0f, s1 = 0.0f;
#pragma unroll
      for (int j = 0; j < NH; ++j) {
        const float d = s_dy[(m - r0) * NH + j];
        if (NH == kNO && j >= kNA) s1 = fmaf(d, w[j], s1); else s0 = fmaf(d, w[j], s0);
        acc[j] = fmaf(d, xv, acc[j]);
      }
      if (NH == kNO) s0 += s1;
      const float dz = s0 * lrelu_mask(xv);
      if (a.dZ != nullptr) a.dZ[(size_t)m * a.H + k] = dz;
      if (a.dZ16 != nullptr) a.dZ16[(size_t)m * a.H + k] = (_Float16)(dz * sc16);
    }
  }
  };
  HEAD_DISPATCH(a.X416 != nullptr, rows_loop);
  if (!want_w) return;
#pragma unroll
  for (int j = 0; j < NH; ++j) s_acc[(rg * NH + j) * 64 + kc] = acc[j];
  __syncthreads();
  float* my_slab = a.slab + ((size_t)rc * nkb + blockIdx.x) * NH * 64;
  if (rg < NH) {
    const int j = rg;
    float v = 0.0f;
#pragma unroll
    for (int g = 0; g < 16; ++g) v += s_acc[(g * NH + j) * 64 + kc];
    slab_st(&my_slab[j * 64 + kc], v);
  }
  if (rg == NH && blockIdx.x == 0 && kc < NH) {
    float v = 0.0f;
    for (int m = 0; m < r1 - r0; ++m) v += s_dy[m * NH + kc];
    slab_st(&a.slab[(size_t)RC * nkb * NH * 64 + rc * 16 + kc], v);
  }
  asm volatile("s_waitcnt vmcnt(0)" ::: "memory");
  __syncthreads();
  if (tid == 0) {
    const int t = __hip_atomic_fetch_add(a.ticket + blockIdx.x, 1, __ATOMIC_RELAXED, __HIP_MEMORY_SCOPE_AGENT);
    s_last = (t == RC - 1);
  }
  __syncthreads();
  if (!s_last) return;
  float ssq = 0.0f;
  if (rg < NH) {
    const int j = rg;
    float v = 0.0f;
    for (int c = 0; c < RC; ++c) v += slab_ld(&a.slab[((size_t)c * nkb + blockIdx.x) * NH * 64 + j * 64 + kc]);
    a.dW[(size_t)j * a.H + k] = v;
    ssq = v * v;
  } else if (rg == NH && blockIdx.x == 0 && kc < NH) {
    float v = 0.0f;
    for (int c = 0; c < RC; ++c) v += slab_ld(&a.slab[(size_t)RC * nkb * NH * 64 + c * 16 + kc]);
    a.db[kc] = v;
    ssq = v * v;
  }
  ssq = wave_sum64(ssq);
  if (kc == 0) s_acc[rg] = ssq;
  __syncthreads();
  if (tid == 0) {
    float t = 0.0f;
#pragma unroll
    for (int g = 0; g <= NH; ++g) t += s_acc[g];
    if (a.partial != nullptr) a.partial[blockIdx.x] = t;
    a.ticket[blockIdx.x] = 0;
  }
}

template <bool F16 = false>
__global__ __launch_bounds__(256) void k_dqda_head_bwd(const DqdaHeadArgs a, const QHeadRider rider) {
  extern __shared__ __attribute__((aligned(16))) float smem[];
  __shared__ float s_d[16][17];
  __shared__ float s_dy[16 * kNO];
  int blk = (int)blockIdx.x;
  if constexpr (F16) asm volatile("" : "+s"(blk) : "s"(a.H), "s"(a.row_tiles), "s"(a.W), "s"(a.X416), "s"(a.aout16), "s"(a.t16.P), "s"(a.t16.Q), "s"(a.t16.ldp), "s"(a.t16.Kred), "s"(a.ls_mult));
  else asm volatile("" : "+s"(blk) : "s"(a.H), "s"(a.row_tiles), "s"(a.W), "s"(a.X4), "s"(a.aout16), "s"(a.pr.P), "s"(a.pr.Q), "s"(a.pr.ldp), "s"(a.pr.Kred));
  const int tiles = a.row_tiles * (a.dxc != nullptr ? 1 : (a.H + 255) >> 8);
  if (blk >= tiles) { q_head_rider(rider, blk - tiles); return; }
  const int rt = blk % a.row_tiles, cc = blk / a.row_tiles;
  const int tid = threadIdx.x, q0 = rt * 16;
  const bool live = (cc << 8) + tid < a.H;
  const int k = live ? (cc << 8) + tid : a.H - 1;
  float wh[kNO], xv[16];
#pragma unroll
  for (int j = 0; j < kNO; ++j) wh[j] = a.W[(size_t)j * a.H + k];
#pragma unroll
  for (int r = 0; r < 16; ++r) xv[r] = F16 ? (float)a.X416[(size_t)(q0 + r) * a.H + k] : a.X4[(size_t)(q0 + r) * a.H + k];
  float out = 0.0f;
  if (tid < 16 * kNO) out = a.aout16[(size_t)(q0 + tid / kNO) * kAP + tid % kNO];
  f32x4 v;
  float sc16 = 0.0f;
  if constexpr (F16) {
    v = dgrad_narrow_tile16<8>(a.t16, rt, smem);
    float inv_ls = a.inv_ls;
    sc16 = a.scale16;
    if (a.ls_mult != nullptr) { inv_ls *= a.ls_mult[1]; sc16 *= a.ls_mult[0]; }
    v.x *= inv_ls; v.y *= inv_ls; v.z *= inv_ls; v.w *= inv_ls;
  }
  else v = dgrad_narrow_tile<8>(a.pr, 0, rt, smem);
  if (tid < 64) {
    const int li = tid & 15, lg = tid >> 4;
    s_d[li][(lg << 2) + 0] = v.x; s_d[li][(lg << 2) + 1] = v.y; s_d[li][(lg << 2) + 2] = v.z; s_d[li][(lg << 2) + 3] = v.w;
  }
  __syncthreads();
  if (a.dxc != nullptr) {
    if (tid < 16 * kNO) a.dxc[(size_t)(q0 + tid / kNO) * a.lddxc + tid % kNO] = s_d[tid / kNO][tid % kNO];
    return;
  }
  if (tid < 16 * kNO) {
    const int r = tid / kNO, j = tid % kNO;
    float d = s_d[r][j];
    float mn, mx;
    inverting_bounds(j, mn, mx);
    if (d < 0) d *= (mx - out) / (mx - mn);
    else if (d > 0) d *= (out - mn) / (mx - mn);
    if (cc == 0) a.dA16[(size_t)(q0 + r) * kAP + j] = d;
    s_dy[tid] = d;
  }
  __syncthreads();
#pragma unroll
  for (int r = 0; r < 16; ++r) {
    float s0 = 0.0f, s1 = 0.0f;
#pragma unroll
    for (int j = 0; j < kNO; ++j) {
      const float d = s_dy[r * kNO + j];
      if (j >= kNA) s1 = fmaf(d, wh[j], s1); else s0 = fmaf(d, wh[j], s0);
    }
    s0 += s1;
    const float dz = s0 * lrelu_mask(xv[r]);
    if (!live) continue;
    if constexpr (F16) a.dZ16[(size_t)(q0 + r) * a.H + k] = (_Float16)(dz * sc16);
    else a.dZ[(size_t)(q0 + r) * a.H + k] = dz;
  }
}
inline hipError_t dqda_head_bwd_launch(DqdaHeadArgs& a, const QHeadRider& rider, const LaunchOn& on) {
  a.row_tiles = a.rows / 16;
  a.pr.tiles_p = 1; a.pr.tiles_q = a.row_tiles; a.pr.tile_base = 0;
  const dim3 grid(a.row_tiles * (a.dxc != nullptr ? 1 : (a.H + 255) / 256) + rider.blocks);
  if (a.dZ16 != nullptr) return launch(on, k_dqda_head_bwd<true>, grid, dim3(256), kNarrowDgradLds, a, rider);
  return launch(on, k_dqda_head_bwd<false>, grid, dim3(256), kNarrowDgradLds, a, rider);
}

template <int NH>
__global__ __launch_bounds__(256) void k_head_bwd_big(HeadBwdBigArgs b) {
  typedef __attribute__((ext_vector_type(4))) _Float16 h4;
  const HeadBwdArgs& a = b.a;
  extern __shared__ __attribute__((aligned(16))) float sm[];
  float* s_dy = sm;
  float* s_red = sm + 64 * NH;
  const int tid = threadIdx.x, w = tid >> 6, lane = tid & 63;
  if (b.chunks > 0 && (int)blockIdx.x >= b.chunks) {
    const float* rW = a.qr_W ? a.qr_W : a.W; const float* rX4 = a.qr_W ? a.qr_X4 : a.X4;
    const _Float16* rX416 = a.qr_W ? a.qr_X416 : a.X416; const int rH = a.qr_W ? a.qr_H : a.H;
    const int nwave = ((int)gridDim.x - b.chunks) * (int)gridDim.y * 4;
    const int wv = (((int)blockIdx.x - b.chunks) * (int)gridDim.y + (int)blockIdx.y) * 4 + w;
    const bool hoist = rH <= 1024;
    f32x4 wreg[4];
    if (hoist) {
#pragma unroll
      for (int t = 0; t < 4; ++t) { const int k = lane * 4 + 256 * t; wreg[t] = k < rH ? *reinterpret_cast<const f32x4*>(rW + k) : f32x4{0.f, 0.f, 0.f, 0.f}; }
    }
    for (int r0 = wv * 4; r0 < a.rows; r0 += nwave * 4) {
      if (hoist) {
        f32x4 xr[4][4];
        if (rX416 != nullptr) {
          head_h4 hr[4][4];
#pragma unroll
          for (int j = 0; j < 4; ++j)
#pragma unroll
            for (int t = 0; t < 4; ++t) {
              const int k = lane * 4 + 256 * t;
              hr[j][t] = (r0 + j < a.rows && k < rH) ? *reinterpret_cast<const head_h4*>(rX416 + (size_t)(r0 + j) * rH + k) : head_h4{(_Float16)0.f, (_Float16)0.f, (_Float16)0.f, (_Float16)0.f};
            }
#pragma unroll
          for (int j = 0; j < 4; ++j)
#pragma unroll
            for (int t = 0; t < 4; ++t) xr[j][t] = f32x4{(float)hr[j][t].x, (float)hr[j][t].y, (float)hr[j][t].z, (float)hr[j][t].w};
        } else {
#pragma unroll
          for (int j = 0; j < 4; ++j)
#pragma unroll
            for (int t = 0; t < 4; ++t) {
              const int k = lane * 4 + 256 * t;
              xr[j][t] = (r0 + j < a.rows && k < rH) ? *reinterpret_cast<const f32x4*>(rX4 + (size_t)(r0 + j) * rH + k) : f32x4{0.f, 0.f, 0.f, 0.f};
            }
        }
#pragma unroll
        for (int j = 0; j < 4; ++j) {
          float acc = 0.0f;
#pragma unroll
          for (int t = 0; t < 4; ++t) {
            acc = fmaf(xr[j][t].x, wreg[t].x, acc); acc = fmaf(xr[j][t].y, wreg[t].y, acc);
            acc = fmaf(xr[j][t].z, wreg[t].z, acc); acc = fmaf(xr[j][t].w, wreg[t].w, acc);
          }
          acc = wave_sum64(acc);
          if (lane == 0 && r0 + j < a.rows) { const float v = acc + a.q_bias[0]; a.q_out[r0 + j] = v; a.qsum_partial[r0 + j] = (double)v; }
        }
      } else {
        for (int j = 0; j < 4 && r0 + j < a.rows; ++j) {
          const size_t x0 = (size_t)(r0 + j) * rH;
          float acc = 0.0f;
          for (int k = lane * 4; k < rH; k += 256) {
            const f32x4 xv = head_ld4(rX4, rX416, x0 + k), wv4 = *reinterpret_cast<const f32x4*>(rW + k);
            acc = fmaf(xv.x, wv4.x, acc); acc = fmaf(xv.y, wv4.y, acc); acc = fmaf(xv.z, wv4.z, acc); acc = fmaf(xv.w, wv4.w, acc);
          }
          acc = wave_sum64(acc);
          if (lane == 0) { const float v = acc + a.q_bias[0]; a.q_out[r0 + j] = v; a.qsum_partial[r0 + j] = (double)v; }
        }
      }
    }
    return;
  }
  const int m0 = blockIdx.x * 64, kb = blockIdx.y * 256, k0 = kb + lane * 4;
  const bool want_w = a.dW != nullptr;
  f32x4 wv[NH], acc[NH];
#pragma unroll
  for (int j = 0; j < NH; ++j) { wv[j] = *reinterpret_cast<const f32x4*>(a.W + (size_t)j * a.H + k0); acc[j] = f32x4{0.f, 0.f, 0.f, 0.f}; }
  f32x4 xr[16];
  head_h4 hr[16];
  if (a.X416 != nullptr) {
#pragma unroll
    for (int r = 0; r < 16; ++r) hr[r] = *reinterpret_cast<const head_h4*>(a.X416 + (size_t)(m0 + w * 16 + r) * a.H + k0);
  } else {
#pragma unroll
    for (int r = 0; r < 16; ++r) xr[r] = *reinterpret_cast<const f32x4*>(a.X4 + (size_t)(m0 + w * 16 + r) * a.H + k0);
  }
  for (int i = tid; i < 64 * NH; i += 256) {
    const int m = m0 + i / NH, j = i % NH;
    float d;
    if constexpr (NH == kNO) {
      d = a.dXc[(size_t)m * a.ldx + a.S + j];
      const float out = a.aout16[(size_t)m * kAP + j];
      float mn, mx;
      inverting_bounds(j, mn, mx);
      if (d < 0) d *= (mx - out) / (mx - mn);
      else if (d > 0) d *= (out - mn) / (mx - mn);
      if (blockIdx.y == 0) a.dA16[(size_t)m * kAP + j] = d;
    } else {
      d = a.dyh ? a.dyh[(size_t)m * a.lddy + j] : -1.0f;
    }
    s_dy[i] = d;
  }
  const float sc16 = b.dZ16 != nullptr ? ls_live(b.scale16, a.ls_mult) : 0.0f;
  __syncthreads();
  if (a.X416 != nullptr) {
#pragma unroll
    for (int r = 0; r < 16; ++r) xr[r] = f32x4{(float)hr[r].x, (float)hr[r].y, (float)hr[r].z, (float)hr[r].w};
  }
#pragma unroll
  for (int r = 0; r < 16; ++r) {
    const int ml = w * 16 + r, m = m0 + ml;
    const f32x4 x = xr[r];
    f32x4 s0 = f32x4{0.f, 0.f, 0.f, 0.f}, s1 = f32x4{0.f, 0.f, 0.f, 0.f};
#pragma unroll
    for (int j = 0; j < NH; ++j) {
      const float d = s_dy[ml * NH + j];
      if (NH == kNO && j >= kNA) { s1.x = fmaf(d, wv[j].x, s1.x); s1.y = fmaf(d, wv[j].y, s1.y); s1.z = fmaf(d, wv[j].z, s1.z); s1.w = fmaf(d, wv[j].w, s1.w); }
      else { s0.x = fmaf(d, wv[j].x, s0.x); s0.y = fmaf(d, wv[j].y, s0.y); s0.z = fmaf(d, wv[j].z, s0.z); s0.w = fmaf(d, wv[j].w, s0.w); }
      acc[j].x = fmaf(d, x.x, acc[j].x); acc[j].y = fmaf(d, x.y, acc[j].y); acc[j].z = fmaf(d, x.z, acc[j].z); acc[j].w = fmaf(d, x.w, acc[j].w);
    }
    if (NH == kNO) { s0.x += s1.x; s0.y += s1.y; s0.z += s1.z; s0.w += s1.w; }
    const f32x4 dz = f32x4{s0.x * lrelu_mask(x.x), s0.y * lrelu_mask(x.y), s0.z * lrelu_mask(x.z), s0.w * lrelu_mask(x.w)};
    if (a.dZ != nullptr) *reinterpret_cast<f32x4*>(a.dZ + (size_t)m * a.H + k0) = dz;
    if (b.dZ16 != nullptr) {
      const h4 hz = h4{(_Float16)(dz.x * sc16), (_Float16)(dz.y * sc16), (_Float16)(dz.z * sc16), (_Float16)(dz.w * sc16)};
      *reinterpret_cast<h4*>(b.dZ16 + (size_t)m * a.H + k0) = hz;
    }
  }
  if (want_w) {
#pragma unroll
    for (int j = 0; j < NH; ++j) *reinterpret_cast<f32x4*>(s_red + ((w * NH + j) * 256 + lane * 4)) = acc[j];
  }
  if (!want_w) return;
  __syncthreads();
  float* slab = b.slab2 + (size_t)blockIdx.x * NH * a.H;
  for (int i = tid; i < NH * 256; i += 256) {
    const int j = i >> 8, c = i & 255;
    slab[(size_t)j * a.H + kb + c] = (s_red[(0 * NH + j) * 256 + c] + s_red[(1 * NH + j) * 256 + c]) +
                                     (s_red[(2 * NH + j) * 256 + c] + s_red[(3 * NH + j) * 256 + c]);
  }
  if (blockIdx.y == 0 && tid < NH) {
    float v = 0.0f;
    for (int m = 0; m < 64; ++m) v += s_dy[m * NH + tid];
    const size_t n_chunks = b.chunks > 0 ? (size_t)b.chunks : (size_t)gridDim.x;
    b.slab2[n_chunks * NH * a.H + blockIdx.x * 16 + tid] = v;
  }
}
template <int NH>
__global__ __launch_bounds__(256) void k_head_wred(HeadBwdBigArgs b, int chunks) {
  const HeadBwdArgs& a = b.a;
  __shared__ float s[4][64];
  __shared__ float s_bias;
  const int j = blockIdx.y, w = threadIdx.x >> 6, lane = threadIdx.x & 63;
  const int k = blockIdx.x * 64 + lane;
  float v = 0.0f;
#pragma unroll 4
  for (int c = w; c < chunks; c += 4) v += b.slab2[((size_t)c * NH + j) * a.H + k];
  s[w][lane] = v;
  if (w == 1) {
    float t = 0.0f;
    if (blockIdx.x == 0) {
      for (int c = lane; c < chunks; c += 64) t += b.slab2[(size_t)chunks * NH * a.H + c * 16 + j];
      t = wave_sum64(t);
      if (lane == 0) a.db[j] = t;
    }
    if (lane == 0) s_bias = t * t;
  }
  __syncthreads();
  if (w != 0) return;
  v = (s[0][lane] + s[1][lane]) + (s[2][lane] + s[3][lane]);
  a.dW[(size_t)j * a.H + k] = v;
  float ssq = v * v;
  ssq = wave_sum64(ssq);
  if (lane == 0 && a.partial != nullptr) a.partial[j * gridDim.x + blockIdx.x] = ssq + s_bias;
}

}
```

### dqn-hfo_amd/csrc/learner_internal.hip.h

```cpp
#pragma once
#include <hip/hip_runtime.h>
#include <rccl/rccl.h>
#include <zlib.h>
#include <unistd.h>

#include <algorithm>
#include <cmath>
#include <cstdarg>
#include <cstdio>
#include <cstdlib>
#include <cstring>
#include <deque>
#include <random>
#include <string>
#include <vector>
#include <mutex>
#include <chrono>
#include <thread>

#include "../../include/dqnhip.h"
#include "../../include/dqnhip_env.h"
#include "gemm_common.hip.h"
#include "learner_args.hip.h"
#include "gemm_plan.hip.h"
#include "hgemm_plan.hip.h"
#include "state_image.h"

namespace dqnhip_host {
using namespace dqnhip;

extern thread_local std::string g_err;

inline int fail(const char* fmt, ...) {
  char buf[1024];
  va_list ap; va_start(ap, fmt); vsnprintf(buf, sizeof buf, fmt, ap); va_end(ap);
  g_err = buf;
  return 1;
}

#define HIPCHK(expr)                                                                  \
  do {                                                                                \
    hipError_t e__ = (expr);                                                          \
    if (e__ != hipSuccess)                                                            \
      return fail("%s failed: %s (%s:%d)", #expr, hipGetErrorString(e__), __FILE__, __LINE__); \
  } while (0)
#define RC(expr) do { int rc__ = (expr); if (rc__) return rc__; } while (0)

inline int round_up(int x, int m) { return (x + m - 1) / m * m; }
inline size_t round_up_z(size_t x, size_t m) { return (x + m - 1) / m * m; }

constexpr int kMaxL = DQNHIP_MAX_HIDDEN;
constexpr int kIxBanks = 2;
constexpr int kIxSizes = 5;
constexpr int kGroupMinRows = 512;

struct NetLayout {
  int L = 0, in_dim = 0, NH = 0;
  int dims[kMaxL + 1] = {0};
  int kp[kMaxL + 1] = {0};
  size_t w_off[kMaxL] = {0}, b_off[kMaxL] = {0}, hw_off = 0, hb_off = 0;
  size_t arena = 0;
  size_t dense = 0;
  int part_off[kMaxL + 1] = {0};
  int part_db = 0;
  int n_part = 0;
};

void layout_init(NetLayout& l, int in_dim, const dqnhip_config& c, bool actor);

enum Family { kFamFwdLds4x2, kFamDgrad, kFamWgrad, kFamAdam, kFamBwdPair, kFamFwdLds2x2, kFamFwdDirect, kFamHgemmFwd, kFamHgemmDgrad, kFamHgemmWgrad,
              kFamPerSync, kFamPerSample, kFamPerUpdate, kNumFamily };
extern const char* const kFamily[kNumFamily];
struct TimingRec { Family family; hipEvent_t a, b; };

enum GraphSlot {
  kGraphSampled,
  kGraphExplicit,
  kGraphPipe0,
  kGraphPipe1,
  kGraphMulti,
  kGraphChainHead,
  kGraphChainPar1,
  kGraphChainPar0,
  kNumGraphSlots
};

struct PerTreeHost { float* lvl[8] = {nullptr}; int n[8] = {0}; int levels = 0; };
struct PerHost {
  dqnhip_per_config cfg{};
  PerTreeHost tree; float* tree_base = nullptr; size_t tree_floats = 0;
  void* dev = nullptr;
  int* idx = nullptr; int* slot = nullptr;
  float *prob = nullptr, *u = nullptr, *w = nullptr, *td_abs = nullptr;
  long long pending = 0; bool changed = false;
  long long syncs = 0;
};
struct DiagHost;
struct StateAsync;

}

using namespace dqnhip;
using namespace dqnhip_host;

struct dqnhip_learner {
  dqnhip_config cfg;
  int B = 0, S = 0, L = 0;
  NetLayout la, lc;
  hipStream_t stream = nullptr;
  bool own_stream = false;
  float* w[4] = {nullptr, nullptr, nullptr, nullptr};
  float* m[2] = {nullptr, nullptr};
  float* v[2] = {nullptr, nullptr};
  float* g[2] = {nullptr, nullptr};
  float* grad_base = nullptr; bool own_grad = false;
  Ring ring{};
  DevState* st = nullptr;
  int* done_counter = nullptr;
  long long h_head = 0, h_size = 0;
  bool ring_stale = false;
  dqnhip_learner* ring_owner = nullptr;
  dqnhip_learner* w_owner = nullptr;
  size_t shared_fl[2] = {0, 0};
  int sharers = 0;
  bool ring_shared = false;
  hipEvent_t ring_ev = nullptr; hipStream_t ring_last = nullptr; bool ring_ev_valid = false;
  std::mutex ring_mu;
  int h_actor_iter = 0, h_critic_iter = 0;
  unsigned long long sample_states_calls = 0;
  ncclComm_t comm = nullptr;
  int rccl_version = 0;
  bool dp_per_layer = false;
  bool dp_half = false;
  bool dp_shard = false;
  float* shard_total = nullptr;
  bool shard_stale = false;
  uint16_t* g16[2] = {nullptr, nullptr};
  float* dp_tails = nullptr;
  hipStream_t comm_stream = nullptr;
  hipEvent_t comm_ev[2] = {nullptr, nullptr};
  hipGraphExec_t dp_graph = nullptr;
  bool dp_graph_failed = false;
  hipGraphExec_t dp_graph_n = nullptr;
  bool dp_graph_n_failed = false;
  int next_phase = 0;
  float* Xa_s = nullptr; float* Xa_n = nullptr; float* Xc_tr = nullptr; float* Xc_pl = nullptr; float* Xc_nx = nullptr;
  float* Xa_s2[2] = {nullptr, nullptr}; float* Xc_pl2[2] = {nullptr, nullptr};
  float* act[5][kMaxL + 1] = {{nullptr}};
  float* dZa[kMaxL + 1] = {nullptr};
  float* dZc[kMaxL + 1] = {nullptr};
  float *mb_reward = nullptr, *mb_mc = nullptr, *mb_term = nullptr;
  float* qdot[2] = {nullptr, nullptr};
  float* Wact_t = nullptr;
  float* Zs = nullptr;
  float* U3 = nullptr;
  int* mb_idx = nullptr;
  int* idx_pinned = nullptr;
  const int* idx_pinned_dev = nullptr;
  float* stats_dev = nullptr;
  float *aout_t16 = nullptr, *aout16 = nullptr, *dA16 = nullptr;
  float *q_t = nullptr, *q1 = nullptr, *q2 = nullptr, *y = nullptr, *dq = nullptr;
  float* loss_partial = nullptr; double* q_partial = nullptr; int n_head_blocks = 0;
  float* part[2] = {nullptr, nullptr};
  float* part_dp = nullptr; int n_part_dp = 0;
  float* head_slab = nullptr; int* head_ticket = nullptr;
  float* head_slab2 = nullptr;
  bool fp16 = false;
  float ls_c = 1.f, ls_q = 1.f, ls_a = 1.f;
  bool ls_dynamic = false;
  int k16[2][kMaxL + 1] = {{0}};
  h16* w16a[4] = {nullptr, nullptr, nullptr, nullptr};
  h16* w16[4][kMaxL] = {{nullptr}};
  h16* act16[5][kMaxL + 1] = {{nullptr}};
  h16* dZ16[2][kMaxL + 1] = {{nullptr}};
  bool w16_dirty[4] = {true, true, true, true};
  std::vector<void*> allocs16;
  bool act_fp16 = false;
  unsigned long long act_epoch = 0;
  h16* actp16[kMaxL + 1] = {nullptr};
  float* actp16_out = nullptr;
  int actp16_rows = 0;
  void* stage_dev = nullptr; size_t stage_bytes = 0;
  float* act_buf = nullptr; size_t act_floats = 0;
  float* pinned_stats = nullptr;
  bool timing = false;
  std::vector<TimingRec> recs;
  int cap_u = -1;
  int cap_n = 16;
  hipGraphExec_t graph_small[3] = {nullptr, nullptr, nullptr};
  hipGraphExec_t graph_exec[kNumGraphSlots] = {nullptr};
  bool graph_failed = false;
  unsigned long long epoch = 0;
  bool chain_cap = false;
  bool chain_valid = false; int chain_par = 0;
  unsigned long long chain_epoch = 0, chain_ring_epoch = 0;
  std::vector<int32_t> chain_idx;
  int* idx_next_pinned[2] = {nullptr, nullptr}; const int* idx_next_dev[2] = {nullptr, nullptr};
  hipEvent_t pipe_ev[2] = {nullptr, nullptr};
  int* pipe_idx_dev[2] = {nullptr, nullptr}; int* pipe_idx_pinned[2] = {nullptr, nullptr};
  float* pipe_stats[2] = {nullptr, nullptr};
  unsigned long long pipe_count = 0;
  int* ix_idx[kIxBanks] = {nullptr}; const int* ix_idx_dev[kIxBanks] = {nullptr};
  float* ix_stats[kIxBanks] = {nullptr}; float* ix_stats_dev[kIxBanks] = {nullptr};
  hipEvent_t ix_ev[kIxBanks] = {nullptr};
  int ix_busy[kIxBanks] = {0};
  int ix_next = 0;
  hipGraphExec_t ix_graph[kIxBanks][kIxSizes] = {{nullptr}};
  long long opt_launches[3] = {0, 0, 0};
  int ix_nodes[kIxSizes] = {0};
  const int* cap_idx = nullptr;
  float* cap_stats = nullptr;
  std::deque<float> ix_pairs;
  std::deque<std::pair<unsigned long long, int>> ix_flagged;
  unsigned long long ix_harvested = 0, ix_collected = 0;
  int ix_prev_flags = 0;
  long long per_env_slack = 0;
  PerHost* per = nullptr;
  DiagHost* diag = nullptr;
  StateAsync* sasync = nullptr;
};

namespace dqnhip_host {

using H = dqnhip_learner;

inline H* RO(H* h) { return h->ring_owner ? h->ring_owner : h; }
inline const H* RO(const H* h) { return h->ring_owner ? h->ring_owner : h; }
inline float* wat(const H* h, int net, size_t off) {
  return ((off < h->shared_fl[net & 1]) ? h->w_owner->w[net] : h->w[net]) + off;
}

struct RingUse {
  H* o; hipStream_t st; bool on;
  RingUse(H* h) : o(RO(h)), st(h->stream), on(RO(h)->ring_shared) {
    if (!on) return;
    o->ring_mu.lock();
    if (o->ring_ev_valid && o->ring_last != st) hipStreamWaitEvent(st, o->ring_ev, 0);
  }
  ~RingUse() {
    if (!on) return;
    hipEventRecord(o->ring_ev, st); o->ring_last = st; o->ring_ev_valid = true;
    o->ring_mu.unlock();
  }
};

inline LaunchOn timed(H* h, Family fam, hipStream_t st) {
  if (!h->timing) return st;
  hipEvent_t a = nullptr, b = nullptr;
  hipEventCreate(&a); hipEventCreate(&b);
  h->recs.push_back({fam, a, b});
  return {st, a, b};
}

void dense_to_arena(const NetLayout& l, const float* dense, std::vector<float>& arena);
void arena_to_dense(const NetLayout& l, const std::vector<float>& arena, float* dense);
inline const NetLayout& layout_of(const H* h, int net) { return (net & 1) ? h->lc : h->la; }
int validate(const dqnhip_config* c);
bool is_pow2(float x);
bool bwd_layer_is_pair(const NetLayout& l, int i, int rows);
bool bwd_is_shifted(const H* h, const NetLayout& l, int rows);
bool head_big_ok(const H* h, int rows, int Hd);
bool dqda_head_shape_ok(const H* h, int panel_w);
bool early_l0(const H* h);
inline size_t grad_arena_floats(const NetLayout& la, const NetLayout& lc) { return la.arena + 64 + lc.arena + 64; }

struct FwdPass { int net; const NetLayout* l; float** act; const float* seed_w = nullptr; float* seed_out = nullptr;
                 const float* dot_w = nullptr; float* dot_out = nullptr; };

int layer_forward(H* h, hipStream_t st, const FwdPass* passes, int n, int rows, int i);
int tower_forward(H* h, hipStream_t st, const FwdPass* passes, int n, int rows, int first_layer = 0);
int tower_forward16_on(H* h, hipStream_t st, int net, h16* const* panels, int rows);
constexpr int kMultiU = 16;
inline uint64_t sample_key(const H* h) { return (uint64_t)h->cfg.seed + 0x9E3779B97F4A7C15ull * (uint64_t)h->cfg.dp_rank; }
inline void shard_range(const H* h, int net, size_t& lo, size_t& hi, int rank = -1) {
  const size_t slice = layout_of(h, net).arena / (size_t)h->cfg.dp_world;
  const size_t r = (size_t)(rank < 0 ? h->cfg.dp_rank : rank);
  lo = r * slice; hi = lo + slice;
}
struct UpdatePlan {
  bool fp16, dp;
  bool shifted_c, shifted_a;
  bool head_rides_c, head_rides_a;
  bool fuse_q;
  bool fused_seed;
  bool fuse_head;
  bool critic_l0;
  bool first_layers_merged;
  bool early_l0;
  bool tails_ride;
  bool prioritized;
};
UpdatePlan plan_of(const H* h);
inline void select_panels(H* h, int par) { h->Xa_s = h->Xa_s2[par]; h->Xc_pl = h->Xc_pl2[par]; h->act[1][0] = h->Xa_s; h->act[4][0] = h->Xc_pl; }
struct NextL0 { ActorL0 a; PlainL0 c, ct; };
int adam_launch(H* h, hipStream_t st, int net, const float* partial, int n_partial, size_t begin, size_t end, const TickArgs* tick = nullptr,
                bool corr_pre = true, const FirstLayerRider* fl = nullptr, const GatherArgs* early_gather = nullptr, const NextL0* next_l0 = nullptr);
int sumsq_launch(H* h, int net, size_t begin = 0, size_t end = 0);
int to_bf16_launch(H* h, int net);
int shard_scal_launch(H* h, float* tail);
int run_phase(H* h, int phase, const int* idx_dev);
int sync_dirty16(H* h);
int prepare_kernels(const H* h);
int refresh_ring(H* h);
int stage_indices(H* h, const int32_t* idx_host, const int** idx_dev);
int run_update(H* h, const int* idx_dev);
struct CaptureSpec {
  int updates = 1; bool multi = false; int of = kMultiU; int chain_pos = -1;
  const int* idx_dev = nullptr;
  const int* idx_bank = nullptr; float* stats_bank = nullptr;
  int (*body)(H*, const int*) = run_update;
};
int capture_updates(H* h, const CaptureSpec& s, hipGraph_t* graph);
int capture_exec(H* h, const CaptureSpec& s, hipGraphExec_t* out, int* kernel_nodes = nullptr);
int ix_harvest_all(H* h);
int ensure_stage(H* h, size_t bytes);
int ensure_act(H* h, int rows);
inline int act16_rows(int n) { return round_up(n, 64); }
inline int act16_width(const H* h, int i) { return std::max(h->k16[0][i], h->k16[1][i]); }
int ensure_act16(H* h, int rows);
void drop_graphs(H* h);
int dp_reduce_slice(H* h, hipStream_t st, int net, size_t off, size_t count);
int dp_allgather_weights(H* h, int net);
int dp_destroy_impl(H* h, bool keep_learner);
const char* rccl_path();
bool same_nets(const H* a, const H* b);
int pack_rows16_launch(hipStream_t st, const float* src, int n, int S, int ld_src, h16* dst, int rows, int k16);
int per_sync_if_needed(H* h);
void per_note_append(H* h, long long n);
int per_sample_launch(H* h);
int per_fill_launch(H* h, const int* idx_dev);
int per_update_launch(H* h);
int per_clear(H* h);
void per_free(H* h);
int per_read_p_max(H* h, float* p_max);
int per_restore(H* h, const float* leaves, int head, int size, float p_max, long long syncs);
int per_refuse(const H* h, const char* what);
void diag_free(H* h);
int state_pack_params_launch(H* h, const dqnhip_state::PackSeg* segs_dev, int n_seg, dqnhip_state::StateRec* rec_dev);
int state_pack_ring_launch(H* h, const dqnhip_state::RingPackArgs& a);
int state_crc_launch(H* h, const dqnhip_state::CrcArgs& a);
int state_async_join(H* h, const char* what);
void state_async_free(H* h);
int snap_pack_replay_launch(H* h, uint8_t* stream_dev);
int snapshot_async_join(H* h, const char* what);

}
```

### include/dqnhip.h

```cpp
#ifndef DQNHIP_H_
#define DQNHIP_H_

#include <stddef.h>
#include <stdint.h>

#ifdef __cplusplus
extern "C" {
#endif

#define DQNHIP_ACTION_SIZE 4
#define DQNHIP_ACTION_PARAM_SIZE 6
#define DQNHIP_ACTOR_OUT 10
#define DQNHIP_MAX_HIDDEN 8

enum dqnhip_net {
  DQNHIP_ACTOR = 0,
  DQNHIP_CRITIC = 1,
  DQNHIP_ACTOR_TARGET = 2,
  DQNHIP_CRITIC_TARGET = 3
};

enum dqnhip_param_kind {
  DQNHIP_KIND_W = 0,
  DQNHIP_KIND_M = 1,
  DQNHIP_KIND_V = 2,
  DQNHIP_KIND_G = 3
};

enum dqnhip_solver {
  DQNHIP_SOLVER_ADAM = 0,
  DQNHIP_SOLVER_SGD = 1,
  DQNHIP_SOLVER_NESTEROV = 2,
  DQNHIP_SOLVER_ADAGRAD = 3,
  DQNHIP_SOLVER_RMSPROP = 4,
  DQNHIP_SOLVER_ADADELTA = 5
};

#define DQNHIP_FP32 0
#define DQNHIP_FP16 1
#define DQNHIP_LOSS_SCALE_STATIC 0
#define DQNHIP_LOSS_SCALE_DYNAMIC 1

typedef struct dqnhip_config {
  int32_t struct_size;
  int32_t minibatch;
  int32_t state_size;
  int32_t num_hidden;
  int32_t hidden[DQNHIP_MAX_HIDDEN];
  int32_t replay_capacity;
  int32_t soft_update_freq;
  double gamma;
  double beta;
  double tau;
  float actor_lr;
  float critic_lr;
  float momentum;
  float momentum2;
  float delta;
  float clip_gradients;
  int32_t device;
  int32_t dp_world;
  int32_t dp_rank;
  int32_t use_graph;
  uint64_t seed;
  void* stream;
  void* grad_arena;
  size_t grad_arena_bytes;
  int32_t precision;
  float loss_scale;
  int32_t solver_type;
  float rms_decay;
  int32_t tuning_flags;
  int32_t loss_scale_mode;
  int32_t loss_scale_growth_interval;
  float loss_scale_min_mult;
  float loss_scale_max_mult;
} dqnhip_config;

#define DQNHIP_TUNE_FP16_WGRAD_PER_LAYER 1
#define DQNHIP_TUNE_SEPARATE_HEAD_SEED 2
#define DQNHIP_TUNE_BWD_UNSHIFTED 4
#define DQNHIP_TUNE_SEPARATE_ACTOR_HEAD_BWD 8
#define DQNHIP_TUNE_SEPARATE_Q_TRAIN 16
#define DQNHIP_TUNE_SEPARATE_FIRST_LAYER 32
#define DQNHIP_TUNE_SEPARATE_CRITIC_FIRST_LAYERS 64
#define DQNHIP_TUNE_LATE_GATHER 128

typedef struct dqnhip_learner* dqnhip_handle;

void dqnhip_default_config(dqnhip_config* cfg, int32_t state_size);

const char* dqnhip_solver_name(int32_t solver_type);

size_t dqnhip_grad_arena_bytes(const dqnhip_config* cfg);

const char* dqnhip_last_error(void);

int dqnhip_create(const dqnhip_config* cfg, dqnhip_handle* out);
int dqnhip_destroy(dqnhip_handle h);


int dqnhip_update(dqnhip_handle h, const int32_t* idx_host,
                  float* critic_loss, float* avg_q);

int dqnhip_update_pipelined(dqnhip_handle h, const int32_t* idx_host,
                            float* critic_loss, float* avg_q);

int dqnhip_update_chained(dqnhip_handle h, const int32_t* idx_host, const int32_t* idx_next,
                          float* critic_loss, float* avg_q);

int dqnhip_update_async(dqnhip_handle h, const int32_t* idx_host);

int dqnhip_update_async_n(dqnhip_handle h, int32_t n);

int dqnhip_update_indexed_n(dqnhip_handle h, const int32_t* idx_host , int32_t n);

int dqnhip_collect_stats(dqnhip_handle h, float* critic_loss , float* avg_q ,
                         int32_t cap, int32_t* n_out);

int dqnhip_update_phase(dqnhip_handle h, int32_t phase, const int32_t* idx_host);
int dqnhip_update_abort(dqnhip_handle h);

int dqnhip_apply_update(dqnhip_handle h, int32_t net);
int dqnhip_apply_update_sharded(dqnhip_handle h, int32_t net, int32_t world);

#define DQNHIP_PLAN_FP16 1
#define DQNHIP_PLAN_DATA_PARALLEL 2
#define DQNHIP_PLAN_BWD_SHIFTED_CRITIC 4
#define DQNHIP_PLAN_BWD_SHIFTED_ACTOR 8
#define DQNHIP_PLAN_HEAD_WGRAD_RIDES_CRITIC 16
#define DQNHIP_PLAN_HEAD_WGRAD_RIDES_ACTOR 32
#define DQNHIP_PLAN_Q_TRAIN_IN_DGRAD 64
#define DQNHIP_PLAN_HEAD_SEED_FUSED 128
#define DQNHIP_PLAN_DQDA_HEAD_BWD 256
#define DQNHIP_PLAN_CRITIC_L0_RIDES 512
#define DQNHIP_PLAN_FIRST_LAYERS_MERGED 1024
#define DQNHIP_PLAN_EARLY_GATHER_L0 2048
#define DQNHIP_PLAN_DP_TAILS_RIDE 4096
#define DQNHIP_PLAN_PRIORITIZED 8192
typedef struct dqnhip_update_plan {
  int32_t struct_size;
  int32_t forms;
  int32_t launches_single;
  int32_t launches_graph_first;
  int32_t launches_in_graph;
  int32_t updates_per_graph;
  int32_t collectives;
  int32_t solver_type;
} dqnhip_update_plan;
int dqnhip_get_update_plan(dqnhip_handle h, dqnhip_update_plan* out);

int dqnhip_grad_buffer(dqnhip_handle h, int32_t net, void** dptr, size_t* nfloats);

#define DQNHIP_DP_ID_BYTES 128
#define DQNHIP_DP_PER_LAYER 1
#define DQNHIP_DP_HALF_GRADS 2
#define DQNHIP_DP_SHARD_OPT 4
#define DQNHIP_DP_UNVERIFIED_OK 256
int dqnhip_dp_info(int32_t* rccl_version, char* path, size_t path_bytes);
int dqnhip_dp_unique_id(void* id_out, size_t bytes);
int dqnhip_dp_init(dqnhip_handle h, const void* id, size_t bytes, int32_t flags);
int dqnhip_dp_init_file(dqnhip_handle h, const char* path, int32_t flags, int32_t timeout_s);
int dqnhip_dp_rendezvous_file(const char* path, int32_t rank, int32_t world, int32_t timeout_s, void* id, size_t bytes);
int dqnhip_dp_rendezvous_cleanup(const char* path, int32_t world);
int dqnhip_dp_graph_active(dqnhip_handle h, int32_t* active);
int dqnhip_dp_broadcast_params(dqnhip_handle h, int32_t root);
int dqnhip_dp_update(dqnhip_handle h, const int32_t* idx_host);
int dqnhip_dp_update_n(dqnhip_handle h, int32_t n);
int dqnhip_dp_gather_state(dqnhip_handle h);
int dqnhip_dp_destroy(dqnhip_handle h);

int dqnhip_read_stats(dqnhip_handle h, float* critic_loss, float* avg_q);
int dqnhip_skipped_steps(dqnhip_handle h, int64_t* count);

typedef struct dqnhip_loss_scale_state {
  int32_t struct_size;
  int32_t mode;
  float mult_critic, mult_actor;
  int32_t good_critic, good_actor;
  int32_t backoffs_critic, backoffs_actor;
  int32_t growths_critic, growths_actor;
  int32_t skipped_steps;
  int32_t reserved;
} dqnhip_loss_scale_state;
int dqnhip_get_loss_scale(dqnhip_handle h, dqnhip_loss_scale_state* out);
int dqnhip_set_loss_scale(dqnhip_handle h, float mult_critic, float mult_actor);

int dqnhip_reduce_gradients_local(dqnhip_handle* learners, int32_t n, int32_t net);

int dqnhip_benchmark(dqnhip_handle h, int32_t warmup, int32_t iterations,
                     float* avg_ms);

int dqnhip_benchmark_blocking(dqnhip_handle h, int32_t warmup, int32_t iterations, uint64_t seed,
                              int32_t pipelined, float* avg_ms);

int dqnhip_select_actions(dqnhip_handle h, const float* states_host, int32_t n,
                          float* actor_out_host);
int dqnhip_select_actions_device(dqnhip_handle h, const float* states_dev,
                                 int32_t n, float* actor_out_dev);
int dqnhip_select_actions_net(dqnhip_handle h, int32_t net,
                              const float* states_host, int32_t n,
                              float* actor_out_host);

int dqnhip_critic_forward(dqnhip_handle h, int32_t net, const float* states_host,
                          const float* actor_out_host, int32_t n, float* q_host);

int dqnhip_set_act_precision(dqnhip_handle h, int32_t precision);
int dqnhip_get_act_precision(dqnhip_handle h, int32_t* precision);

int dqnhip_add_transitions(dqnhip_handle h, const float* states, const float* actor_out,
                           const float* rewards, const float* on_policy_targets,
                           const float* next_states, const uint8_t* terminal, int32_t n);
int dqnhip_add_transition(dqnhip_handle h, const float* state, const float* actor_out,
                          float reward, float on_policy_target,
                          const float* next_state, uint8_t terminal);
int dqnhip_add_transitions_device(dqnhip_handle h, const float* states, const float* actor_out,
                                  const float* rewards, const float* on_policy_targets,
                                  const float* next_states, const uint8_t* terminal, int32_t n);

int dqnhip_label_transitions(double gamma, const float* rewards, int32_t n,
                             float* on_policy_targets);

int dqnhip_sample_states(dqnhip_handle h, const int32_t* idx_host, int32_t n, float* states_host);
int dqnhip_get_actor_output(dqnhip_handle h, int32_t net, int32_t batch_size, float* actor_out_host);

int dqnhip_memory_size(dqnhip_handle h, int32_t* size);
int dqnhip_clear_memory(dqnhip_handle h);
int dqnhip_read_memory(dqnhip_handle h, int32_t first, int32_t n, float* states,
                       float* actor_out, float* rewards, float* on_policy_targets,
                       float* next_states, uint8_t* terminal);

int dqnhip_snapshot_replay_memory(dqnhip_handle h, const char* filename);
int dqnhip_load_replay_memory(dqnhip_handle h, const char* filename);


int dqnhip_param_count(dqnhip_handle h, int32_t net, size_t* count);
int dqnhip_get_params(dqnhip_handle h, int32_t net, int32_t kind, float* host, size_t count);
int dqnhip_set_params(dqnhip_handle h, int32_t net, int32_t kind, const float* host, size_t count);
int dqnhip_clone_to_target(dqnhip_handle h, int32_t net);
int dqnhip_get_iters(dqnhip_handle h, int32_t* actor_iter, int32_t* critic_iter);
int dqnhip_set_iters(dqnhip_handle h, int32_t actor_iter, int32_t critic_iter);

int dqnhip_share_parameters(dqnhip_handle owner, dqnhip_handle other, int32_t num_actor_layers,
                            int32_t num_critic_layers);
int dqnhip_share_replay_memory(dqnhip_handle owner, dqnhip_handle other);

int dqnhip_get_config(dqnhip_handle h, dqnhip_config* out);

int dqnhip_save_caffemodel(dqnhip_handle h, int32_t net, const char* filename);
int dqnhip_load_caffemodel(dqnhip_handle h, int32_t net, const char* filename);
int dqnhip_solver_snapshot(dqnhip_handle h, int32_t net, const char* prefix, int32_t* iter_out);
int dqnhip_solver_restore(dqnhip_handle h, int32_t net, const char* solverstate);
int dqnhip_snapshot(dqnhip_handle h, const char* save_path, const char* snapshot_prefix,
                    int32_t remove_old, int32_t snapshot_memory);
int dqnhip_snapshot_async(dqnhip_handle h, const char* save_path, const char* snapshot_prefix, int32_t remove_old, int32_t snapshot_memory,
                          int32_t compress_threads);
int dqnhip_snapshot_wait(dqnhip_handle h, int32_t* actor_iter, int32_t* critic_iter);
int dqnhip_snapshot_poll(dqnhip_handle h, int32_t* done);
int dqnhip_find_latest_snapshot(const char* snapshot_prefix, char* actor, char* critic, char* memory,
                                size_t buf_len);
int dqnhip_find_hiscore(const char* snapshot_prefix, int32_t* score);
int dqnhip_remove_files_matching_regexp(const char* regexp);
int dqnhip_files_matching_regexp(const char* regexp, char* buf, size_t buf_len, int32_t* count);
int dqnhip_remove_snapshots(const char* regexp, int32_t min_iter);


int dqnhip_debug_read(dqnhip_handle h, const char* name, float* host, size_t count);

int dqnhip_get_stream(dqnhip_handle h, void** stream);
int dqnhip_set_kernel_timing(dqnhip_handle h, int32_t enable);
int dqnhip_get_kernel_timing(dqnhip_handle h, const char* family, float* avg_ms,
                             int64_t* launches, int32_t reset);

typedef struct dqnhip_diag_moments {
  int64_t count, n_zero, n_nonfinite;
  double sum_abs, sum_sq;
  float max_abs, reserved;
} dqnhip_diag_moments;
#define DQNHIP_DIAG_BINS 64
typedef struct dqnhip_diag_blob {
  int32_t net, layer, is_bias, reserved;
  dqnhip_diag_moments w, g, lag, step;
  int32_t g_hist[DQNHIP_DIAG_BINS];
} dqnhip_diag_blob;
typedef struct dqnhip_diag_panel {
  int32_t pass, layer, rows, cols;
  int64_t n_negative;
  int32_t dead_units, reserved;
  dqnhip_diag_moments a;
  int32_t hist[DQNHIP_DIAG_BINS];
} dqnhip_diag_panel;
typedef struct dqnhip_diag_row { float min, max; double sum, sum_sq; int64_t n_nonfinite; } dqnhip_diag_row;
typedef struct dqnhip_diag_action { float min, max; double sum; int64_t n_out_of_bounds; } dqnhip_diag_action;
#define DQNHIP_DIAG_MAX_BLOBS (2 * (2 * DQNHIP_MAX_HIDDEN + 4))
#define DQNHIP_DIAG_MAX_PANELS (5 * DQNHIP_MAX_HIDDEN)
typedef struct dqnhip_diag_report {
  int32_t struct_size;
  int32_t n_blobs, n_panels, has_per;
  dqnhip_diag_blob blobs[DQNHIP_DIAG_MAX_BLOBS];
  dqnhip_diag_panel panels[DQNHIP_DIAG_MAX_PANELS];
  dqnhip_diag_row q_target, y, q_train, q_policy, td;
  int64_t n_terminal;
  dqnhip_diag_action actor_out[DQNHIP_ACTOR_OUT];
  double dq_da_sum_abs;
  float dq_da_max_abs;
  float per_w_min;
  double per_w_sum;
  float per_prob_min, per_td_abs_max;
  int32_t actor_iter, critic_iter;
  float critic_loss, avg_q;
  double grad_norm[2], clip_scale[2];
  int32_t fp16, loss_scale_mode;
  float loss_scale_critic, loss_scale_dqda, loss_scale_actor;
  float mult_critic, mult_actor;
  int32_t reserved;
} dqnhip_diag_report;
int dqnhip_diag_collect(dqnhip_handle h, dqnhip_diag_report* out);


typedef struct dqnhip_per_config {
  int32_t struct_size;
  float alpha;
  float beta0;
  int32_t beta_anneal_iters;
  float eps;
  uint64_t seed;
} dqnhip_per_config;
void dqnhip_per_default_config(dqnhip_per_config* cfg);

int dqnhip_per_enable(dqnhip_handle h, const dqnhip_per_config* cfg);

typedef struct dqnhip_per_state {
  int32_t struct_size;
  int32_t enabled;
  int32_t levels;
  int32_t size;
  float total, p_max, beta_now, reserved;
  uint64_t next_counter;
  int64_t syncs;
} dqnhip_per_state;
int dqnhip_per_get_state(dqnhip_handle h, dqnhip_per_state* out);

int dqnhip_per_get_priorities(dqnhip_handle h, int32_t first, int32_t n, float* leaf_host);
int dqnhip_per_set_priorities(dqnhip_handle h, int32_t first, int32_t n, const float* leaf_host);

int dqnhip_per_sample(dqnhip_handle h, uint64_t counter, int32_t n_batches, int32_t* idx_host, float* prob_host);

int dqnhip_per_debug_read(dqnhip_handle h, const char* name, float* host, size_t count);

#define DQNHIP_STATE_NO_MEMORY 1
int dqnhip_save_state(dqnhip_handle h, const char* filename, int32_t flags,
                      const void* user, size_t user_bytes);
int dqnhip_load_state(dqnhip_handle h, const char* filename);
typedef struct dqnhip_state_info {
  int32_t struct_size;
  int32_t version, flags, precision, minibatch, state_size, num_hidden, hidden[DQNHIP_MAX_HIDDEN], replay_capacity, memory_size,
      actor_iter, critic_iter, has_memory, has_per, has_loss_scale;
  uint64_t seed, update_counter, user_bytes, file_bytes;
  int32_t solver_type;
  float rms_decay;
} dqnhip_state_info_t;
int dqnhip_state_info(const char* filename, dqnhip_state_info_t* out);
int dqnhip_state_read_user(const char* filename, void* buf, size_t cap, size_t* n_out);

int dqnhip_save_state_async(dqnhip_handle h, const char* filename, int32_t flags, const void* user, size_t user_bytes);
int dqnhip_save_state_wait(dqnhip_handle h);
int dqnhip_save_state_poll(dqnhip_handle h, int32_t* done);
int dqnhip_state_crc32_device(dqnhip_handle h, const void* host_bytes, size_t bytes, int32_t misalign, uint32_t* crc);



#ifdef __cplusplus
}
#endif
#endif
```

Baseline: 3652 updates/s.

## Pass hot GEMM and head arguments as leading scalar kernel params for kernarg preload

Adds a compact 14-dword preload record (pointers, leading dims, tile counts, magic divisor, split) as leading scalar kernel parameters for the fwd/dgrad LDS GEMMs, wgrad tail, q-train dgrad, head forward and dqda head kernels. The aim is for the hardware to preload these words into user SGPRs so each block can decode its tile without waiting on the scalar load of the kernarg struct. The original struct-based path stays as a fallback when the record does not fit, or when a new tuning flag disables it. Costs are more kernel variants of the entry logic, duplicated parameter passing and extra host-side packing.

```diff
diff --git a/dqn-hfo_amd/capi.py b/dqn-hfo_amd/capi.py
--- a/dqn-hfo_amd/capi.py
+++ b/dqn-hfo_amd/capi.py
@@ -15,6 +15,7 @@
 TUNE_SEPARATE_FIRST_LAYER = 32
 TUNE_SEPARATE_CRITIC_FIRST_LAYERS = 64
 TUNE_LATE_GATHER = 128
+TUNE_NO_KERNARG_PRELOAD = 256
 PLAN_FORMS = ("fp16", "data_parallel", "bwd_shifted_critic", "bwd_shifted_actor", "head_wgrad_rides_critic", "head_wgrad_rides_actor",
               "q_train_in_dgrad", "head_seed_fused", "dqda_head_bwd", "critic_l0_rides", "first_layers_merged", "early_gather_l0", "dp_tails_ride", "prioritized")
 LOSS_SCALE_STATIC, LOSS_SCALE_DYNAMIC = 0, 1
diff --git a/dqn-hfo_amd/csrc/gemm_bodies.hip.h b/dqn-hfo_amd/csrc/gemm_bodies.hip.h
--- a/dqn-hfo_amd/csrc/gemm_bodies.hip.h
+++ b/dqn-hfo_amd/csrc/gemm_bodies.hip.h
@@ -107,6 +107,77 @@
   HotArgs<N> r;
   const int b = request_args(a, r, (int)blockIdx.x);
   return problem_of_tile(a, r, b, tile_p, tile_q);
+}
+
+struct PreTile { int pi, tile_p, tile_q, tiles_p, tiles_q, tile_base; const float* P; const float* Q; };
+__host__ __device__ __forceinline__ PreTile preload_decode(const GemmPreload& w, int b) {
+  PreTile t;
+  const int split = (int)(w.flags >> kPreSplitShift);
+  t.pi = b >= split ? 1 : 0;
+  t.tile_base = t.pi ? split : 0;
+  t.tiles_p = (int)(w.tiles & ((1u << kPreTilesQShift) - 1)); t.tiles_q = (int)(w.tiles >> kPreTilesQShift);
+  tile_decode(t.tiles_p, t.tiles_q, w.magic, b - t.tile_base, t.tile_p, t.tile_q);
+  t.P = t.pi ? w.P1 : w.P0; t.Q = t.pi ? w.Q1 : w.Q0;
+  return t;
+}
+struct PreRecordTile { bool mine; int tile_p, tile_q, tiles_p, tiles_q; };
+__host__ __device__ __forceinline__ PreRecordTile preload_record_decode(const GemmPreload& w, int b) {
+  PreRecordTile t;
+  const int bb = b - (int)(w.flags >> kPreSplitShift);
+  t.tiles_p = (int)(w.tiles & ((1u << kPreTilesQShift) - 1)); t.tiles_q = (int)(w.tiles >> kPreTilesQShift);
+  t.mine = bb >= 0 && bb < t.tiles_p * t.tiles_q;
+  tile_decode(t.tiles_p, t.tiles_q, w.magic, t.mine ? bb : 0, t.tile_p, t.tile_q);
+  return t;
+}
+inline bool preload_record_fits(const GemmHot& h, int tiles_p, int tiles_q) {
+  return h.ldp >= 0 && h.ldp <= kMaxLeadingDim && h.ldq >= 0 && h.ldq <= kMaxLeadingDim && h.Kred >= 0 &&
+         tile_magic_covers(tiles_p, tiles_q) && tiles_p < (1 << kPreTilesQShift) && tiles_q < (1 << (32 - kPreTilesQShift)) &&
+         h.tq_magic == tile_magic(tiles_q);
+}
+template <int N>
+inline GemmPreload make_preload_words(const GemmArgs<N>& a, int i, uint32_t split_or_first) {
+  GemmPreload w{};
+  if (i < 0 || i >= N || i >= a.head.n || split_or_first > kPreNoSplit) return w;
+  const GemmHot& h = a.hot[i];
+  const int tp = a.head.tiles_p[i], tq = a.head.tiles_q[i];
+  if (!preload_record_fits(h, tp, tq)) return w;
+  w.P0 = h.P; w.Q0 = h.Q; w.ldp = (uint32_t)h.ldp; w.ldq = (uint32_t)h.ldq; w.Kred = (uint32_t)h.Kred;
+  w.tiles = (uint32_t)tp | (uint32_t)tq << kPreTilesQShift; w.magic = h.tq_magic;
+  w.flags = kPreValid | split_or_first << kPreSplitShift;
+  return w;
+}
+template <int N>
+inline GemmPreload make_preload_record(const GemmArgs<N>& a, int i, bool off, int first = 0) {
+  if (off || first < 0) return GemmPreload{};
+  return make_preload_words(a, i, (uint32_t)first);
+}
+template <int N>
+inline GemmPreload make_preload_grouped(const GemmArgs<N>& a, bool off) {
+  if (off || a.head.tile_base[0] != 0) return GemmPreload{};
+  if (a.head.n == 1) return make_preload_words(a, 0, kPreNoSplit);
+  if (N < 2 || a.head.n != 2) return GemmPreload{};
+  const GemmHot &h = a.hot[0], &g = a.hot[N > 1 ? 1 : 0];
+  const int tp = a.head.tiles_p[0], tq = a.head.tiles_q[0], split = a.head.tile_base[1];
+  if (g.ldp != h.ldp || g.ldq != h.ldq || g.Kred != h.Kred || a.head.tiles_p[1] != tp || a.head.tiles_q[1] != tq || g.tq_magic != h.tq_magic) return GemmPreload{};
+  if (split < 0 || (uint32_t)split >= kPreNoSplit) return GemmPreload{};
+  GemmPreload w = make_preload_words(a, 0, (uint32_t)split);
+  if (!(w.flags & kPreValid) || split != tp * tq) return GemmPreload{};
+  w.P1 = g.P; w.Q1 = g.Q;
+  return w;
+}
+template <int N>
+__device__ __forceinline__ GemmProblem problem_of_preload(const GemmPreload& w, const GemmArgs<N>& a, int b, int& tile_p, int& tile_q) {
+  const PreTile t = preload_decode(w, b);
+  tile_p = t.tile_p; tile_q = t.tile_q;
+  const int pi = N == 1 ? 0 : t.pi;
+  const GemmHot& h = a.hot[pi];
+  return make_problem(t.P, t.Q, h.C, (int)w.ldp, (int)w.ldq, h.ldc, h.Pdim, h.Qdim, (int)w.Kred, h.mode, a.cold[pi], t.tiles_p, t.tiles_q, t.tile_base);
+}
+template <int I, int N>
+__device__ __forceinline__ GemmProblem record_of_preload(const GemmPreload& w, const GemmArgs<N>& a, const PreRecordTile& t) {
+  static_assert(I < N, "record not carried");
+  const GemmHot& h = a.hot[I];
+  return make_problem(w.P0, w.Q0, h.C, (int)w.ldp, (int)w.ldq, h.ldc, h.Pdim, h.Qdim, (int)w.Kred, h.mode, a.cold[I], t.tiles_p, t.tiles_q, a.head.tile_base[I]);
 }
 
 template <int NACC>
diff --git a/dqn-hfo_amd/csrc/gemm_common.hip.h b/dqn-hfo_amd/csrc/gemm_common.hip.h
--- a/dqn-hfo_amd/csrc/gemm_common.hip.h
+++ b/dqn-hfo_amd/csrc/gemm_common.hip.h
@@ -63,9 +63,26 @@
 };
 static_assert(sizeof(GemmHeader) == 64 && sizeof(GemmHot) == 64, "one 16-dword scalar load each");
 
+struct GemmPreload {
+  const float* P0; const float* Q0; const float* P1; const float* Q1;
+  uint32_t ldp, ldq, Kred;
+  uint32_t tiles;
+  uint32_t magic;
+  uint32_t flags;
+};
+static_assert(sizeof(GemmPreload) == 14 * 4, "16 user SGPRs less the kernarg pointer");
+constexpr uint32_t kPreValid = 1;
+constexpr int kPreSplitShift = 2, kPreTilesQShift = 20;
+constexpr uint32_t kPreNoSplit = (1u << (32 - kPreSplitShift)) - 1;
+#define DQN_PRELOAD_PARAMS const float* pre_P0, const float* pre_Q0, const float* pre_P1, const float* pre_Q1, \
+    uint32_t pre_ldp, uint32_t pre_ldq, uint32_t pre_Kred, uint32_t pre_tiles, uint32_t pre_magic, uint32_t pre_flags
+#define DQN_PRELOAD_WORDS(pre) (pre).P0, (pre).Q0, (pre).P1, (pre).Q1, (pre).ldp, (pre).ldq, (pre).Kred, (pre).tiles, (pre).magic, (pre).flags
+#define DQN_PRELOAD_BLOCK GemmPreload{pre_P0, pre_Q0, pre_P1, pre_Q1, pre_ldp, pre_ldq, pre_Kred, pre_tiles, pre_magic, pre_flags}
+
 struct LaunchOn {
   hipStream_t stream;
   hipEvent_t start = nullptr, stop = nullptr;
+  bool no_preload = false;
   LaunchOn(hipStream_t s) : stream(s) {}
   LaunchOn(hipStream_t s, hipEvent_t t0, hipEvent_t t1) : stream(s), start(t0), stop(t1) {}
 };
diff --git a/dqn-hfo_amd/csrc/gemm_direct.hip.h b/dqn-hfo_amd/csrc/gemm_direct.hip.h
--- a/dqn-hfo_amd/csrc/gemm_direct.hip.h
+++ b/dqn-hfo_amd/csrc/gemm_direct.hip.h
@@ -18,10 +18,15 @@
   fwd_direct_body<TP, TQ>(pr, tile_p, tile_q, smem);
 }
 template <int TP, int TQ, bool PIN, int NSLOT = 2>
-__global__ __launch_bounds__(256) void gemm_fwd_lds(const GemmArgs<kMaxGroup> args) {
-  extern __shared__ __attribute__((aligned(16))) float smem[];
-  int tile_p, tile_q;
-  const GemmProblem pr = problem_of_block(args, tile_p, tile_q);
+__global__ __launch_bounds__(256) void gemm_fwd_lds(DQN_PRELOAD_PARAMS, const GemmArgs<kMaxGroup> args) {
+  extern __shared__ __attribute__((aligned(16))) float smem[];
+  int tile_p, tile_q;
+  if (!(pre_flags & kPreValid)) {
+    const GemmProblem pr = problem_of_block(args, tile_p, tile_q);
+    fwd_lds_body<TP, TQ, PIN, NSLOT>(pr, tile_p, tile_q, smem);
+    return;
+  }
+  const GemmProblem pr = problem_of_preload(DQN_PRELOAD_BLOCK, args, (int)blockIdx.x, tile_p, tile_q);
   fwd_lds_body<TP, TQ, PIN, NSLOT>(pr, tile_p, tile_q, smem);
 }
 template <int TPB, int TQ>
@@ -37,10 +42,15 @@
   dgrad_lds_body<TPB, TQ, SCH, DgradNoHook>(pr, tile_p, tile_q, smem, nullptr, none);
 }
 template <int TPB, int TQ>
-__global__ __launch_bounds__(256) void gemm_dgrad_lds(const GemmArgs<kMaxGroup> args) {
-  extern __shared__ __attribute__((aligned(16))) float smem[];
-  int tile_p, tile_q;
-  const GemmProblem pr = problem_of_block(args, tile_p, tile_q);
+__global__ __launch_bounds__(256) void gemm_dgrad_lds(DQN_PRELOAD_PARAMS, const GemmArgs<kMaxGroup> args) {
+  extern __shared__ __attribute__((aligned(16))) float smem[];
+  int tile_p, tile_q;
+  if (!(pre_flags & kPreValid)) {
+    const GemmProblem pr = problem_of_block(args, tile_p, tile_q);
+    dgrad_lds_body<TPB, TQ>(pr, tile_p, tile_q, smem);
+    return;
+  }
+  const GemmProblem pr = problem_of_preload(DQN_PRELOAD_BLOCK, args, (int)blockIdx.x, tile_p, tile_q);
   dgrad_lds_body<TPB, TQ>(pr, tile_p, tile_q, smem);
 }
 template <int TPB, int TQB>
@@ -120,8 +130,16 @@
 }
 
 template <int NH>
-__global__ __launch_bounds__(256) void gemm_wgrad_tail(const GemmArgs<2> args, const HeadWgradRider rider, const TailsArgs tails) {
-  extern __shared__ __attribute__((aligned(16))) float smem[];
+__global__ __launch_bounds__(256) void gemm_wgrad_tail(DQN_PRELOAD_PARAMS, const GemmArgs<2> args, const HeadWgradRider rider, const TailsArgs tails) {
+  extern __shared__ __attribute__((aligned(16))) float smem[];
+  if (pre_flags & kPreValid) {
+    const PreRecordTile t = preload_record_decode(DQN_PRELOAD_BLOCK, (int)blockIdx.x);
+    if (t.mine) {
+      const GemmProblem p1 = record_of_preload<0>(DQN_PRELOAD_BLOCK, args, t);
+      wgrad_direct_body<1, 1>(p1, t.tile_p, t.tile_q, smem);
+      return;
+    }
+  }
   HotArgs<2> r;
   int blk = request_args(args, r, (int)blockIdx.x, tails.on, rider.blocks);
   int tile_p, tile_q;
@@ -190,6 +208,14 @@
   tile_batch(batch, BP, BQ);
   return packed_launch(kernel, batch, 0, lds_bytes, on);
 }
+template <typename K>
+inline hipError_t preload_launch(K kernel, GemmBatch& batch, int BP, int BQ, int lds_bytes, const LaunchOn& on) {
+  tile_batch(batch, BP, BQ);
+  GemmArgs<kMaxGroup> args;
+  if (!pack_args(batch, args)) return hipErrorInvalidValue;
+  const GemmPreload pre = make_preload_grouped(args, on.no_preload);
+  return launch(on, kernel, dim3(batch.total_tiles), dim3(256), lds_bytes, DQN_PRELOAD_WORDS(pre), args);
+}
 
 template <int TP, int TQ>
 constexpr int fwd_direct_lds_bytes() { return 4 * TP * TQ * 64 * 16; }
@@ -203,7 +229,7 @@
 }
 template <int TP, int TQ, bool PIN, int NSLOT = 2>
 inline hipError_t fwd_lds_launch(GemmBatch& b, const LaunchOn& on) {
-  return packed_launch(gemm_fwd_lds<TP, TQ, PIN, NSLOT>, b, 16 * TP, 16 * TQ, (fwd_lds_bytes<TP, TQ, PIN, NSLOT>()), on);
+  return preload_launch(gemm_fwd_lds<TP, TQ, PIN, NSLOT>, b, 16 * TP, 16 * TQ, (fwd_lds_bytes<TP, TQ, PIN, NSLOT>()), on);
 }
 template <int TPB, int TQ>
 constexpr int dgrad_direct_lds_bytes() { return 4 * TPB * 4 * TQ * 64 * 16; }
@@ -215,7 +241,7 @@
 constexpr int dgrad_lds_bytes() { return 4 * ((2 * TQ * 512 > TPB * 4 * TQ * 256) ? 2 * TQ * 512 : TPB * 4 * TQ * 256) * 4; }
 template <int TPB, int TQ>
 inline hipError_t dgrad_lds_launch(GemmBatch& b, const LaunchOn& on) {
-  return packed_launch(gemm_dgrad_lds<TPB, TQ>, b, 64 * TPB, 16 * TQ, dgrad_lds_bytes<TPB, TQ>(), on);
+  return preload_launch(gemm_dgrad_lds<TPB, TQ>, b, 64 * TPB, 16 * TQ, dgrad_lds_bytes<TPB, TQ>(), on);
 }
 template <int TPB, int TQB>
 inline hipError_t wgrad_direct_launch(GemmBatch& b, const LaunchOn& on) {
@@ -271,7 +297,8 @@
   if (lds > (size_t)kWgradTailLdsMax) return hipErrorInvalidValue;
   GemmArgs<2> args;
   if (batch.n != 2 || !pack_args(batch, args)) return hipErrorInvalidValue;
-  return launch(on, gemm_wgrad_tail<NH>, dim3(grid), dim3(256), lds, args, rider, tails);
+  const GemmPreload pre = make_preload_record(args, 0, on.no_preload, rider.blocks + w0.tiles_p * w0.tiles_q);
+  return launch(on, gemm_wgrad_tail<NH>, dim3(grid), dim3(256), lds, DQN_PRELOAD_WORDS(pre), args, rider, tails);
 }
 template <bool DLDS>
 inline hipError_t bwd_seq_launch(GemmBatch& batch, const LaunchOn& on) {
diff --git a/dqn-hfo_amd/csrc/head_fwd_kernels.hip.h b/dqn-hfo_amd/csrc/head_fwd_kernels.hip.h
--- a/dqn-hfo_amd/csrc/head_fwd_kernels.hip.h
+++ b/dqn-hfo_amd/csrc/head_fwd_kernels.hip.h
@@ -4,18 +4,29 @@
 
 namespace dqnhip {
 
-template <int NH, int MODE, bool L1 = false>
-__global__ __launch_bounds__(256) void k_head_fwd(HeadArgs2 a2) {
-  const HeadArgs& a = a2.p[blockIdx.y];
+struct HeadFwdPreload { const float* W0; const float* W1; const float* b0; const float* b1; uint32_t H0, H1, flags; };
+#define DQN_HEAD_PRELOAD_PARAMS const float* pre_W0, const float* pre_W1, const float* pre_b0, const float* pre_b1, \
+    uint32_t pre_H0, uint32_t pre_H1, uint32_t pre_flags
+#define DQN_HEAD_PRELOAD_WORDS(w) (w).W0, (w).W1, (w).b0, (w).b1, (w).H0, (w).H1, (w).flags
+inline HeadFwdPreload make_head_preload(const HeadArgs2& a2, bool two, bool off) {
+  HeadFwdPreload w{};
+  if (off || a2.p[0].H < 1 || (two && a2.p[1].H < 1)) return w;
+  w.W0 = a2.p[0].W; w.b0 = a2.p[0].b; w.H0 = (uint32_t)a2.p[0].H;
+  if (two) { w.W1 = a2.p[1].W; w.b1 = a2.p[1].b; w.H1 = (uint32_t)a2.p[1].H; }
+  w.flags = kPreValid;
+  return w;
+}
+template <int NH, int MODE, bool L1>
+__device__ __forceinline__ void head_fwd_block(const HeadArgs& a, const float* W, const float* b, const int H) {
   const int wave = threadIdx.x >> 6, lane = threadIdx.x & 63;
   __shared__ float s_acc[4][NH];
-  const bool hoist = a.H <= 1024;
-  const float bias_j = threadIdx.x < NH ? a.b[threadIdx.x] : 0.0f;
+  const bool hoist = H <= 1024;
+  const float bias_j = threadIdx.x < NH ? b[threadIdx.x] : 0.0f;
   f32x4 wreg[NH];
   if (hoist) {
 #pragma unroll
     for (int j = 0; j < NH; ++j)
-      wreg[j] = (threadIdx.x * 4 < a.H) ? *reinterpret_cast<const f32x4*>(a.W + (size_t)j * a.H + threadIdx.x * 4) : f32x4{0.f, 0.f, 0.f, 0.f};
+      wreg[j] = (threadIdx.x * 4 < H) ? *reinterpret_cast<const f32x4*>(W + (size_t)j * H + threadIdx.x * 4) : f32x4{0.f, 0.f, 0.f, 0.f};
   }
   constexpr bool kL1 = (L1 && MODE == HEAD_ACTOR && NH == kNO);
   __shared__ float s_mu[kAP];
@@ -40,11 +51,11 @@
     f32x4 zs = f32x4{0.f, 0.f, 0.f, 0.f};
     if constexpr (kL1) { if (l1_on) zs = *reinterpret_cast<const f32x4*>(a.l1_zs + (size_t)row * a.l1_ld + threadIdx.x * 4); }
     auto dots = [&](auto tag) {
-      for (int k = threadIdx.x * 4; k < a.H; k += 1024) {
+      for (int k = threadIdx.x * 4; k < H; k += 1024) {
         const f32x4 xv = head_ld4t<decltype(tag)::value>(a.X, a.X16, x0 + k);
 #pragma unroll
         for (int j = 0; j < NH; ++j) {
-          const f32x4 wv = hoist ? wreg[j] : *reinterpret_cast<const f32x4*>(a.W + (size_t)j * a.H + k);
+          const f32x4 wv = hoist ? wreg[j] : *reinterpret_cast<const f32x4*>(W + (size_t)j * H + k);
           acc[j] = fmaf(xv.x, wv.x, acc[j]); acc[j] = fmaf(xv.y, wv.y, acc[j]);
           acc[j] = fmaf(xv.z, wv.z, acc[j]); acc[j] = fmaf(xv.w, wv.w, acc[j]);
         }
@@ -92,6 +103,13 @@
     }
   }
 }
+template <int NH, int MODE, bool L1 = false>
+__global__ __launch_bounds__(256) void k_head_fwd(DQN_HEAD_PRELOAD_PARAMS, HeadArgs2 a2) {
+  const HeadArgs& a = a2.p[blockIdx.y];
+  if (!(pre_flags & kPreValid)) { head_fwd_block<NH, MODE, L1>(a, a.W, a.b, a.H); return; }
+  const bool second = blockIdx.y != 0;
+  head_fwd_block<NH, MODE, L1>(a, second ? pre_W1 : pre_W0, second ? pre_b1 : pre_b0, (int)(second ? pre_H1 : pre_H0));
+}
 
 template <int NH, int MODE>
 __global__ __launch_bounds__(256) void k_head_fwd_rows(HeadArgs2 a2) {
@@ -182,10 +200,11 @@
       return 0;
     }
   }
+  const HeadFwdPreload w = make_head_preload(a2, b != nullptr, (h->cfg.tuning_flags & DQNHIP_TUNE_NO_KERNARG_PRELOAD) != 0);
   if (a.l1_y != nullptr || (b && b->l1_y != nullptr))
-    HIPCHK(launch(st, k_head_fwd<NH, MODE, true>, dim3(std::min(a.rows, 1024), b ? 2 : 1), dim3(256), 0, a2));
+    HIPCHK(launch(st, k_head_fwd<NH, MODE, true>, dim3(std::min(a.rows, 1024), b ? 2 : 1), dim3(256), 0, DQN_HEAD_PRELOAD_WORDS(w), a2));
   else
-    HIPCHK(launch(st, k_head_fwd<NH, MODE, false>, dim3(std::min(a.rows, 1024), b ? 2 : 1), dim3(256), 0, a2));
+    HIPCHK(launch(st, k_head_fwd<NH, MODE, false>, dim3(std::min(a.rows, 1024), b ? 2 : 1), dim3(256), 0, DQN_HEAD_PRELOAD_WORDS(w), a2));
   return 0;
 }
 
diff --git a/dqn-hfo_amd/csrc/head_kernels.hip.h b/dqn-hfo_amd/csrc/head_kernels.hip.h
--- a/dqn-hfo_amd/csrc/head_kernels.hip.h
+++ b/dqn-hfo_amd/csrc/head_kernels.hip.h
@@ -178,15 +178,7 @@
     if (owner && lane == 0) a.loss_partial[(q0 >> 2) + wave] = ((d2[0] + d2[1]) + d2[2]) + d2[3];
   }
 };
-template <int UNUSED = 0>
-__global__ __launch_bounds__(256) __attribute__((amdgpu_waves_per_eu(1, 1))) void k_dgrad_qtrain(const GemmArgs<1> args, const HeadTrainArgs a) {
-  extern __shared__ __attribute__((aligned(16))) float smem[];
-  __shared__ float s_scale[16], s_dq[16];
-  int tile_p, tile_q;
-  HotArgs<1> r;
-  const int b = request_args(args, r, (int)blockIdx.x);
-  const GemmProblem pr = problem_at<0>(args, r);
-  tile_of_record<0>(r, b, tile_p, tile_q);
+__device__ __forceinline__ void dgrad_qtrain_block(const GemmProblem& pr, const int tile_p, const int tile_q, const HeadTrainArgs& a, float* smem, float* s_scale, float* s_dq) {
   const int q0 = tile_q * 16;
   QTrainHook hook(a, s_scale, s_dq, q0, tile_p);
   dgrad_lds_body<1, 1, true, QTrainHook>(pr, tile_p, tile_q, smem, s_scale, hook);
@@ -202,12 +194,30 @@
     *reinterpret_cast<f32x4*>(a.dZ + x0) = dz;
   }
 }
+template <int UNUSED = 0>
+__global__ __launch_bounds__(256) __attribute__((amdgpu_waves_per_eu(1, 1))) void k_dgrad_qtrain(DQN_PRELOAD_PARAMS, const GemmArgs<1> args, const HeadTrainArgs a) {
+  extern __shared__ __attribute__((aligned(16))) float smem[];
+  __shared__ float s_scale[16], s_dq[16];
+  int tile_p, tile_q;
+  if (!(pre_flags & kPreValid)) {
+    HotArgs<1> r;
+    const int b = request_args(args, r, (int)blockIdx.x);
+    const GemmProblem pr = problem_at<0>(args, r);
+    tile_of_record<0>(r, b, tile_p, tile_q);
+    dgrad_qtrain_block(pr, tile_p, tile_q, a, smem, s_scale, s_dq);
+    return;
+  }
+  const PreRecordTile t = preload_record_decode(DQN_PRELOAD_BLOCK, (int)blockIdx.x);
+  const GemmProblem pr = record_of_preload<0>(DQN_PRELOAD_BLOCK, args, t);
+  dgrad_qtrain_block(pr, t.tile_p, t.tile_q, a, smem, s_scale, s_dq);
+}
 inline hipError_t dgrad_qtrain_launch(GemmBatch& batch, const HeadTrainArgs& a, const LaunchOn& on) {
   batch.n = 1;
   tile_batch(batch, 64, 16);
   GemmArgs<1> args;
   if (!pack_args(batch, args)) return hipErrorInvalidValue;
-  return launch(on, k_dgrad_qtrain<0>, dim3(batch.total_tiles), dim3(256), dgrad_lds_bytes<1, 1>(), args, a);
+  const GemmPreload pre = make_preload_record(args, 0, on.no_preload);
+  return launch(on, k_dgrad_qtrain<0>, dim3(batch.total_tiles), dim3(256), dgrad_lds_bytes<1, 1>(), DQN_PRELOAD_WORDS(pre), args, a);
 }
 
 __device__ __forceinline__ void slab_st(float* p, float v) { __hip_atomic_store(p, v, __ATOMIC_RELAXED, __HIP_MEMORY_SCOPE_AGENT); }
@@ -351,27 +361,51 @@
   }
 }
 
-template <bool F16 = false>
-__global__ __launch_bounds__(256) void k_dqda_head_bwd(const DqdaHeadArgs a, const QHeadRider rider) {
-  extern __shared__ __attribute__((aligned(16))) float smem[];
-  __shared__ float s_d[16][17];
-  __shared__ float s_dy[16 * kNO];
-  int blk = (int)blockIdx.x;
-  if constexpr (F16) asm volatile("" : "+s"(blk) : "s"(a.H), "s"(a.row_tiles), "s"(a.W), "s"(a.X416), "s"(a.aout16), "s"(a.t16.P), "s"(a.t16.Q), "s"(a.t16.ldp), "s"(a.t16.Kred), "s"(a.ls_mult));
-  else asm volatile("" : "+s"(blk) : "s"(a.H), "s"(a.row_tiles), "s"(a.W), "s"(a.X4), "s"(a.aout16), "s"(a.pr.P), "s"(a.pr.Q), "s"(a.pr.ldp), "s"(a.pr.Kred));
-  const int tiles = a.row_tiles * (a.dxc != nullptr ? 1 : (a.H + 255) >> 8);
-  if (blk >= tiles) { q_head_rider(rider, blk - tiles); return; }
-  const int rt = blk % a.row_tiles, cc = blk / a.row_tiles;
+struct DqdaPreload {
+  const float* W; const float* X4; const float* aout16; const float* P; const float* Q;
+  uint32_t ldp, ldq;
+  uint32_t h_kred;
+  uint32_t route;
+};
+static_assert(sizeof(DqdaPreload) == 14 * 4, "16 user SGPRs less the kernarg pointer");
+#define DQN_DQDA_PRELOAD_PARAMS const float* pre_W, const float* pre_X4, const float* pre_aout16, const float* pre_P, const float* pre_Q, \
+    uint32_t pre_ldp, uint32_t pre_ldq, uint32_t pre_h_kred, uint32_t pre_route
+#define DQN_DQDA_PRELOAD_WORDS(w) (w).W, (w).X4, (w).aout16, (w).P, (w).Q, (w).ldp, (w).ldq, (w).h_kred, (w).route
+struct DqdaFirst { int H, row_tiles, tiles; const float* W; const float* X4; const float* aout16; };
+__host__ __device__ __forceinline__ DqdaFirst dqda_preload_decode(const DqdaPreload& w) {
+  DqdaFirst f;
+  f.H = (int)(w.h_kred & 0xFFFFu);
+  f.row_tiles = (int)((w.route >> 1) & 0xFFFFu);
+  f.tiles = f.row_tiles * (int)(w.route >> 17);
+  f.W = w.W; f.X4 = w.X4; f.aout16 = w.aout16;
+  return f;
+}
+inline DqdaPreload make_dqda_preload(const DqdaHeadArgs& a, int row_tiles, bool off) {
+  DqdaPreload w{};
+  const int chunks = a.dxc != nullptr ? 1 : (a.H + 255) / 256;
+  if (off || a.dZ16 != nullptr || a.X4 == nullptr) return w;
+  if (a.H < 1 || a.H > 0xFFFF || a.pr.Kred < 0 || a.pr.Kred > 0xFFFF || row_tiles < 1 || row_tiles > 0xFFFF || chunks > 0x7FFF) return w;
+  if (a.pr.ldp < 0 || a.pr.ldp > kMaxLeadingDim || a.pr.ldq < 0 || a.pr.ldq > kMaxLeadingDim) return w;
+  w.W = a.W; w.X4 = a.X4; w.aout16 = a.aout16; w.P = a.pr.P; w.Q = a.pr.Q;
+  w.ldp = (uint32_t)a.pr.ldp; w.ldq = (uint32_t)a.pr.ldq;
+  w.h_kred = (uint32_t)a.H | (uint32_t)a.pr.Kred << 16;
+  w.route = kPreValid | (uint32_t)row_tiles << 1 | (uint32_t)chunks << 17;
+  return w;
+}
+template <bool F16>
+__device__ __forceinline__ void dqda_head_block(const DqdaHeadArgs& a, const DqdaFirst& f, const GemmProblem& pr, const int blk,
+                                                float* smem, float (*s_d)[17], float* s_dy) {
+  const int rt = blk % f.row_tiles, cc = blk / f.row_tiles;
   const int tid = threadIdx.x, q0 = rt * 16;
-  const bool live = (cc << 8) + tid < a.H;
-  const int k = live ? (cc << 8) + tid : a.H - 1;
+  const bool live = (cc << 8) + tid < f.H;
+  const int k = live ? (cc << 8) + tid : f.H - 1;
   float wh[kNO], xv[16];
 #pragma unroll
-  for (int j = 0; j < kNO; ++j) wh[j] = a.W[(size_t)j * a.H + k];
-#pragma unroll
-  for (int r = 0; r < 16; ++r) xv[r] = F16 ? (float)a.X416[(size_t)(q0 + r) * a.H + k] : a.X4[(size_t)(q0 + r) * a.H + k];
+  for (int j = 0; j < kNO; ++j) wh[j] = f.W[(size_t)j * f.H + k];
+#pragma unroll
+  for (int r = 0; r < 16; ++r) xv[r] = F16 ? (float)a.X416[(size_t)(q0 + r) * f.H + k] : f.X4[(size_t)(q0 + r) * f.H + k];
   float out = 0.0f;
-  if (tid < 16 * kNO) out = a.aout16[(size_t)(q0 + tid / kNO) * kAP + tid % kNO];
+  if (tid < 16 * kNO) out = f.aout16[(size_t)(q0 + tid / kNO) * kAP + tid % kNO];
   f32x4 v;
   float sc16 = 0.0f;
   if constexpr (F16) {
@@ -381,7 +415,7 @@
     if (a.ls_mult != nullptr) { inv_ls *= a.ls_mult[1]; sc16 *= a.ls_mult[0]; }
     v.x *= inv_ls; v.y *= inv_ls; v.z *= inv_ls; v.w *= inv_ls;
   }
-  else v = dgrad_narrow_tile<8>(a.pr, 0, rt, smem);
+  else v = dgrad_narrow_tile<8>(pr, 0, rt, smem);
   if (tid < 64) {
     const int li = tid & 15, lg = tid >> 4;
     s_d[li][(lg << 2) + 0] = v.x; s_d[li][(lg << 2) + 1] = v.y; s_d[li][(lg << 2) + 2] = v.z; s_d[li][(lg << 2) + 3] = v.w;
@@ -413,16 +447,43 @@
     s0 += s1;
     const float dz = s0 * lrelu_mask(xv[r]);
     if (!live) continue;
-    if constexpr (F16) a.dZ16[(size_t)(q0 + r) * a.H + k] = (_Float16)(dz * sc16);
-    else a.dZ[(size_t)(q0 + r) * a.H + k] = dz;
-  }
+    if constexpr (F16) a.dZ16[(size_t)(q0 + r) * f.H + k] = (_Float16)(dz * sc16);
+    else a.dZ[(size_t)(q0 + r) * f.H + k] = dz;
+  }
+}
+template <bool F16 = false>
+__global__ __launch_bounds__(256) void k_dqda_head_bwd(DQN_DQDA_PRELOAD_PARAMS, const DqdaHeadArgs a, const QHeadRider rider) {
+  extern __shared__ __attribute__((aligned(16))) float smem[];
+  __shared__ float s_d[16][17];
+  __shared__ float s_dy[16 * kNO];
+  if constexpr (!F16) {
+    if (pre_route & kPreValid) {
+      const DqdaPreload w{pre_W, pre_X4, pre_aout16, pre_P, pre_Q, pre_ldp, pre_ldq, pre_h_kred, pre_route};
+      const DqdaFirst f = dqda_preload_decode(w);
+      const int blk = (int)blockIdx.x;
+      if (blk >= f.tiles) { q_head_rider(rider, blk - f.tiles); return; }
+      GemmProblem pr = a.pr;
+      pr.P = w.P; pr.Q = w.Q; pr.ldp = (int)w.ldp; pr.ldq = (int)w.ldq; pr.Kred = (int)(w.h_kred >> 16);
+      dqda_head_block<false>(a, f, pr, blk, smem, s_d, s_dy);
+      return;
+    }
+  }
+  int blk = (int)blockIdx.x;
+  if constexpr (F16) asm volatile("" : "+s"(blk) : "s"(a.H), "s"(a.row_tiles), "s"(a.W), "s"(a.X416), "s"(a.aout16), "s"(a.t16.P), "s"(a.t16.Q), "s"(a.t16.ldp), "s"(a.t16.Kred), "s"(a.ls_mult));
+  else asm volatile("" : "+s"(blk) : "s"(a.H), "s"(a.row_tiles), "s"(a.W), "s"(a.X4), "s"(a.aout16), "s"(a.pr.P), "s"(a.pr.Q), "s"(a.pr.ldp), "s"(a.pr.Kred));
+  DqdaFirst f;
+  f.H = a.H; f.row_tiles = a.row_tiles; f.tiles = a.row_tiles * (a.dxc != nullptr ? 1 : (a.H + 255) >> 8);
+  f.W = a.W; f.X4 = a.X4; f.aout16 = a.aout16;
+  if (blk >= f.tiles) { q_head_rider(rider, blk - f.tiles); return; }
+  dqda_head_block<F16>(a, f, a.pr, blk, smem, s_d, s_dy);
 }
 inline hipError_t dqda_head_bwd_launch(DqdaHeadArgs& a, const QHeadRider& rider, const LaunchOn& on) {
   a.row_tiles = a.rows / 16;
   a.pr.tiles_p = 1; a.pr.tiles_q = a.row_tiles; a.pr.tile_base = 0;
   const dim3 grid(a.row_tiles * (a.dxc != nullptr ? 1 : (a.H + 255) / 256) + rider.blocks);
-  if (a.dZ16 != nullptr) return launch(on, k_dqda_head_bwd<true>, grid, dim3(256), kNarrowDgradLds, a, rider);
-  return launch(on, k_dqda_head_bwd<false>, grid, dim3(256), kNarrowDgradLds, a, rider);
+  const DqdaPreload w = make_dqda_preload(a, a.row_tiles, on.no_preload);
+  if (a.dZ16 != nullptr) return launch(on, k_dqda_head_bwd<true>, grid, dim3(256), kNarrowDgradLds, DQN_DQDA_PRELOAD_WORDS(w), a, rider);
+  return launch(on, k_dqda_head_bwd<false>, grid, dim3(256), kNarrowDgradLds, DQN_DQDA_PRELOAD_WORDS(w), a, rider);
 }
 
 template <int NH>
diff --git a/dqn-hfo_amd/csrc/learner_internal.hip.h b/dqn-hfo_amd/csrc/learner_internal.hip.h
--- a/dqn-hfo_amd/csrc/learner_internal.hip.h
+++ b/dqn-hfo_amd/csrc/learner_internal.hip.h
@@ -245,11 +245,12 @@
 };
 
 inline LaunchOn timed(H* h, Family fam, hipStream_t st) {
-  if (!h->timing) return st;
-  hipEvent_t a = nullptr, b = nullptr;
-  hipEventCreate(&a); hipEventCreate(&b);
-  h->recs.push_back({fam, a, b});
-  return {st, a, b};
+  LaunchOn on(st);
+  on.no_preload = (h->cfg.tuning_flags & DQNHIP_TUNE_NO_KERNARG_PRELOAD) != 0;
+  if (!h->timing) return on;
+  hipEventCreate(&on.start); hipEventCreate(&on.stop);
+  h->recs.push_back({fam, on.start, on.stop});
+  return on;
 }
 
 void dense_to_arena(const NetLayout& l, const float* dense, std::vector<float>& arena);
diff --git a/include/dqnhip.h b/include/dqnhip.h
--- a/include/dqnhip.h
+++ b/include/dqnhip.h
@@ -85,6 +85,7 @@
 #define DQNHIP_TUNE_SEPARATE_FIRST_LAYER 32
 #define DQNHIP_TUNE_SEPARATE_CRITIC_FIRST_LAYERS 64
 #define DQNHIP_TUNE_LATE_GATHER 128
+#define DQNHIP_TUNE_NO_KERNARG_PRELOAD 256
 
 typedef struct dqnhip_learner* dqnhip_handle;
 
```

After: 3738 updates/s, median of 6. 1.02x the previous value.
